# duyhominhnguyen/conan-fgw

Hardware: AMD Instinct MI355X
Metric: molecules/s (K=5 conformers) (higher is better)
Workload: dtype f32

## Files before the change

### conan-fgw_amd/_lib.py

```python
from __future__ import annotations

import ctypes
import os
import subprocess

import torch

_HERE = os.path.dirname(os.path.abspath(__file__))
_SO = os.path.join(_HERE, "libconan_fgw_hip.so")
_LIB = None
ABI_VERSION = 6

c_int, c_float, c_void_p, c_ll = ctypes.c_int, ctypes.c_float, ctypes.c_void_p, ctypes.c_longlong


class FgwParams(ctypes.Structure):
    _fields_ = [("alpha", c_float), ("epsilon", c_float), ("max_iter", c_int), ("tol", c_float), ("inner_tol", c_float),
                ("num_iter_max", c_int), ("stop_thr", c_float), ("fixed_structure", c_int), ("fixed_features", c_int),
                ("warmstart", c_int), ("loss_fun", c_int), ("cs_small_int", c_int)]


class BatchLayout(ctypes.Structure):
    _fields_ = [(n, c_int) for n in ("B", "K", "num_graphs", "num_atoms", "num_bond_edges", "max_nodes", "x_dim", "ea_dim")] + \
               [(n, c_ll) for n in ("off_atom_off", "off_bond_off", "off_z", "off_pos", "off_x", "off_bsrc", "off_bdst", "off_battr", "off_y", "bytes")]


class WgradJob(ctypes.Structure):
    _fields_ = [("ws", c_void_p), ("dW", c_void_p), ("dbias", c_void_p), ("M", c_int), ("K", c_int), ("N", c_int), ("slices", c_int)]


class WgradSlabJob(ctypes.Structure):
    _fields_ = [("g", c_void_p), ("x", c_void_p), ("m_dev", c_void_p), ("ws", c_void_p), ("M", c_int), ("K", c_int), ("N", c_int), ("slices", c_int)]


_P = c_void_p
SIGNATURES = {
    "conan_abi_version": (c_int, []),
    "conan_collate_layout": (c_int, [c_int, c_int, _P, _P, c_int, c_int, ctypes.POINTER(BatchLayout)]),
    "conan_collate_pack": (c_int, [ctypes.POINTER(BatchLayout), _P, _P, _P, _P, _P, _P, _P, _P, _P]),
    "conan_collate_unpack": (c_int, [_P, ctypes.POINTER(BatchLayout), _P, _P, _P, _P, _P, _P, _P, _P, _P, _P, _P]),
    "conan_graph_ptr_from_batch": (c_int, [_P, c_int, c_int, _P, _P]),
    "conan_radius_graph_csr": (c_int, [_P, _P, c_int, c_int, c_float, c_int, c_int, _P, _P, _P, _P, _P, _P]),
    "conan_csr_transpose": (c_int, [_P, c_int, c_int, _P, _P, _P, _P, _P, _P]),
    "conan_edge_pairs": (c_int, [_P, _P, _P, _P, _P, c_int, _P, _P, _P, _P, _P, _P, _P, _P]),
    "conan_radius_graph_build_ws": (c_ll, [c_int, c_int, c_int, c_int]),
    "conan_radius_graph_build": (c_int, [_P, _P, c_int, c_int, c_float, c_int, c_int] + [_P] * 12 + [_P]),
    "conan_edge_index_i64": (c_int, [_P, _P, c_int, _P, _P]),
    "conan_embedding_fwd": (c_int, [_P, _P, c_int, c_int, c_int, _P, _P]),
    "conan_onehot_rows": (c_int, [_P, c_int, c_int, c_int, _P, _P]),
    "conan_embedding_bwd_ws": (c_ll, [c_int, c_int, c_int]),
    "conan_embedding_bwd": (c_int, [_P, _P, c_int, c_int, c_int, c_int, _P, _P, _P]),
    "conan_linear_fwd": (c_int, [_P, _P, _P, _P, c_int, c_int, c_int, c_int, c_int, _P, _P, _P]),
    "conan_linear_multi_fwd": (c_int, [_P, _P, _P, c_int, c_int, c_int, c_int, c_int, _P, _P, _P, _P]),
    "conan_linear_sum_fwd": (c_int, [_P, _P, _P, c_int, c_int, _P, _P, c_int, c_int, _P, _P, _P]),
    "conan_ssp_bwd": (c_int, [_P, _P, c_int, c_int, _P, _P, _P]),
    "conan_linear_wgrad_ws": (c_ll, [c_int, c_int, c_int]),
    "conan_linear_wgrad": (c_int, [_P, _P, c_int, c_int, c_int, _P, _P, _P, _P, _P]),
    "conan_bond_graph_csr": (c_int, [_P, c_int, c_int, _P, _P, _P, _P, _P, _P, _P, _P]),
    "conan_gat_edge_vec": (c_int, [_P, _P, c_int, c_int, _P, _P]),
    "conan_gat_edge_vec_bwd": (c_int, [_P, _P, _P, c_int, c_int, _P, _P, _P]),
    "conan_gat_node_alpha": (c_int, [_P, _P, _P, c_int, c_int, _P, _P, _P]),
    "conan_gat_aggregate_fwd": (c_int, [_P, _P, _P, _P, _P, _P, _P, c_int, _P, _P, c_float, c_int, c_int, _P, _P, _P, _P]),
    "conan_gat_bwd_ws": (c_ll, [c_int, c_int, c_int, c_int]),
    "conan_gat_aggregate_bwd": (c_int, [_P] * 15 + [c_int, _P, c_float, c_int, c_int, c_int, _P, _P, _P, _P]),
    "conan_linear_act_fwd": (c_int, [_P, _P, _P, c_int, c_int, c_int, c_int, _P, _P, _P, _P]),
    "conan_unary_fwd": (c_int, [_P, c_ll, c_int, _P, _P]),
    "conan_unary_bwd": (c_int, [_P, _P, c_ll, c_int, _P, _P]),
    "conan_zero_tail": (c_int, [_P, _P, c_int, c_int, _P]),
    "conan_rbf_wgrad": (c_int, [_P, _P, c_int, _P, c_int, c_float, c_int, _P, _P, _P, _P, _P]),
    "conan_wgrad_batchable": (c_int, [c_int, c_int]),
    "conan_linear_wgrad_scaled": (c_int, [_P, _P, c_int, c_int, c_int, _P, _P, _P, _P, _P, _P]),
    "conan_linear_wgrad_slabs": (c_int, [_P, _P, c_int, c_int, c_int, _P, _P, _P]),
    "conan_rbf_wgrad_slabs": (c_int, [_P, _P, c_int, _P, c_int, c_float, c_int, _P, _P, _P]),
    "conan_wgrad_reduce_batch": (c_int, [ctypes.POINTER(WgradJob), c_int, _P]),
    "conan_linear_wgrad_slabs_batch": (c_int, [ctypes.POINTER(WgradSlabJob), c_int, _P]),
    "conan_filter_bwd_supported": (c_int, [c_int, c_int]),
    "conan_filter_bwd_slices": (c_int, [c_int]),
    "conan_filter_bwd_ws": (c_ll, [c_int, c_int, c_int]),
    "conan_filter_bwd": (c_int, [_P, _P, _P, c_int, _P, c_int, c_float, _P, c_int, _P, _P, _P, _P, _P, _P]),
    "conan_filter_bwd2_supported": (c_int, [c_int, c_int]),
    "conan_filter_bwd2_slices": (c_int, [c_int]),
    "conan_filter_bwd2_ws": (c_ll, [c_int, c_int, c_int]),
    "conan_filter_bwd2": (c_int, [_P, _P, _P, c_int, _P, c_int, c_float, _P, c_int, _P, _P, _P, _P, _P, _P, _P, _P]),
    "conan_rbf_fwd": (c_int, [_P, _P, c_int, _P, c_int, c_float, _P, _P]),
    "conan_cutoff_scale": (c_int, [_P, _P, c_int, c_int, c_float, _P, _P, _P]),
    "conan_stage2_head_supported": (c_int, [c_int]),
    "conan_mse_loss_fwd": (c_int, [_P, _P, c_int, _P, _P, _P]),
    "conan_bce_loss_fwd": (c_int, [_P, _P, _P, c_int, c_int, _P, _P, _P]),
    "conan_stage2_head_fwd": (c_int, [_P, _P, _P, _P, _P, _P, _P, _P, _P, c_float, c_int, c_int, c_int, _P, _P, _P, _P, _P]),
    "conan_stage2_head_bwd": (c_int, [_P, _P, _P, _P, _P, _P, _P, c_float, c_int, c_int, c_int, _P, _P, _P, _P, _P, _P, _P, _P, _P, _P]),
    "conan_stage2_head_sums_supported": (c_int, [c_int, c_int, c_int]),
    "conan_stage2_head_sums_fwd": (c_int, [_P] * 10 + [c_float] + [c_int] * 5 + [_P] * 5),
    "conan_stage2_head_sums_bwd": (c_int, [_P] * 8 + [c_float] + [c_int] * 5 + [_P] * 10),
    "conan_adam_flat_step": (c_int, [_P, _P, _P, _P, _P, _P, c_ll] + [ctypes.c_double] * 5 + [_P, _P]),
    "conan_grad_clip_flat": (c_int, [_P, c_ll, ctypes.c_double, _P, _P, _P, _P]),
    "conan_mlp2_supported": (c_int, [c_int, c_int, c_int, c_int]),
    "conan_mlp2_fwd": (c_int, [_P, _P, _P, _P, _P, _P, c_int, c_int, c_int, c_int, _P, _P, _P]),
    "conan_mlp2_bwd": (c_int, [_P, _P, _P, _P, c_int, c_int, c_int, c_int, _P, _P, _P]),
    "conan_mlp2_outact_supported": (c_int, [c_int, c_int, c_int, c_int]),
    "conan_mlp2_outact_fwd": (c_int, [_P, _P, _P, _P, _P, c_int, c_int, c_int, c_int, _P, _P, _P]),
    "conan_mlp2_outact_bwd": (c_int, [_P, _P, _P, _P, c_int, c_int, c_int, c_int, _P, _P, _P, _P]),
    "conan_mlp2_outact_dual_fwd": (c_int, [_P] * 9 + [c_int] * 4 + [_P, c_int, _P, _P, _P, _P, _P]),
    "conan_mlp2_outact_dual_bwd": (c_int, [_P] * 8 + [c_int] * 4 + [_P, _P, _P, _P, _P, _P, _P]),
    "conan_filter_fused_supported": (c_int, [c_int, c_int]),
    "conan_filter_fwd": (c_int, [_P, _P, c_int, _P, c_int, c_float, c_float, c_int, _P, _P, _P, _P, _P, _P, _P]),
    "conan_filter_cfconv_fwd_supported": (c_int, [c_int, c_int]),
    "conan_filter_cfconv_fwd": (c_int, [_P, _P, _P, _P, _P, c_int, _P, c_int, c_float, c_float, c_int, _P, _P, _P, _P, c_int, _P, _P]),
    "conan_cfconv_fwd": (c_int, [_P, _P, _P, _P, _P, c_int, c_int, _P, _P, _P]),
    "conan_cfconv_bwd_xw_pairs_supported": (c_int, [c_int]),
    "conan_cfconv_bwd_xw_pairs": (c_int, [_P] * 10 + [ctypes.c_float, c_int, c_int, _P, _P, _P, _P]),
    "conan_cfconv_bwd_x": (c_int, [_P, _P, _P, _P, _P, _P, c_int, c_int, _P, _P, _P]),
    "conan_cfconv_bwd_w_pairs": (c_int, [_P, _P, _P, c_int, _P, _P, _P, _P, c_int, _P, c_float, _P, _P, _P]),
    "conan_cfconv_bwd_w": (c_int, [_P, _P, _P, c_int, _P, _P, c_int, _P, c_float, _P, _P]),
    "conan_segment_sum_fwd": (c_int, [_P, _P, c_int, c_int, _P, _P]),
    "conan_segment_sum_bwd": (c_int, [_P, _P, c_int, c_int, _P, _P]),
    "conan_visnet_edge_unit": (c_int, [_P, _P, _P, _P, c_int, _P, _P]),
    "conan_visnet_expnormal": (c_int, [_P, _P, c_int, _P, _P, c_int, c_float, c_float, _P, _P]),
    "conan_visnet_neighbor_scale": (c_int, [_P, _P, _P, _P, _P, c_int, c_int, c_float, _P]),
    "conan_visnet_neighbor_scale_to": (c_int, [_P, _P, _P, _P, _P, c_int, c_int, c_float, _P, _P]),
    "conan_concat2": (c_int, [_P, c_int, _P, c_int, c_ll, _P, _P]),
    "conan_visnet_edge_embed": (c_int, [_P, _P, _P, _P, _P, c_int, c_int, _P, _P]),
    "conan_layernorm_fwd": (c_int, [_P, _P, _P, c_int, c_int, c_float, _P, _P]),
    "conan_scale_channels": (c_int, [_P, _P, c_ll, c_int, _P, _P]),
    "conan_scale_channels_add": (c_int, [_P, _P, _P, c_ll, c_int, _P, _P]),
    "conan_visnet_vecdot": (c_int, [_P, c_int, c_int, _P, _P]),
    "conan_visnet_attn_message": (c_int, [_P, _P, _P, _P, _P, _P, _P, _P, c_float, c_int, c_int, c_int, c_int, _P, _P, _P]),
    "conan_visnet_vec_aggregate": (c_int, [_P, _P, _P, _P, _P, c_int, c_int, c_int, _P, _P]),
    "conan_visnet_node_update": (c_int, [_P, _P, _P, _P, _P, _P, c_int, c_int, _P, _P, _P]),
    "conan_visnet_edge_update": (c_int, [_P, _P, _P, _P, _P, _P, _P, c_int, c_int, c_int, _P, _P, _P]),
    "conan_visnet_spatial_norm": (c_int, [_P, c_int, c_int, _P, _P]),
    "conan_visnet_gate": (c_int, [_P, _P, c_int, c_int, c_int, _P, _P, _P]),
    "conan_visnet_prior": (c_int, [_P, _P, _P, _P, c_int, c_int, _P, _P]),
    "conan_silu_fwd": (c_int, [_P, c_int, c_int, _P, _P, _P]),
    "conan_silu_bwd": (c_int, [_P, _P, c_int, c_int, _P, _P, _P]),
    "conan_split2": (c_int, [_P, c_int, c_int, c_ll, _P, _P, _P]),
    "conan_rowsum": (c_int, [_P, c_int, c_int, _P, _P]),
    "conan_scale_scalar": (c_int, [_P, _P, c_ll, _P, _P]),
    "conan_visnet_edge_embed_bwd": (c_int, [_P, _P, _P, _P, _P, _P, _P, _P, _P, c_int, c_int, c_int, _P, _P, _P]),
    "conan_layernorm_bwd_ws": (c_ll, [c_int, c_int]),
    "conan_layernorm_bwd": (c_int, [_P, _P, _P, c_int, c_int, c_float, _P, _P, _P, _P, _P]),
    "conan_layernorm_bwd_res": (c_int, [_P, _P, _P, _P, c_int, c_int, c_float, _P, _P, _P, _P, _P]),
    "conan_visnet_vecdot_bwd": (c_int, [_P, _P, c_int, c_int, _P, _P]),
    "conan_visnet_attn_message_bwd": (c_int, [_P] * 13 + [c_float, c_int, c_int, c_int, c_int] + [_P] * 6),
    "conan_visnet_vec_aggregate_bwd": (c_int, [_P, _P, _P, _P, _P, _P, _P, _P, _P, c_int, c_int, c_int, c_int, _P, _P, _P]),
    "conan_visnet_node_update_bwd": (c_int, [_P, _P, _P, _P, _P, c_int, c_int, _P, _P, _P, _P]),
    "conan_visnet_edge_update_bwd": (c_int, [_P, _P, _P, _P, _P, _P, _P, _P, _P, _P, c_int, c_int, c_int, _P, _P, _P, _P]),
    "conan_visnet_spatial_norm_bwd": (c_int, [_P, _P, c_int, c_int, _P, _P]),
    "conan_visnet_gate_bwd": (c_int, [_P, _P, _P, _P, c_int, c_int, c_int, _P, _P, _P]),
    "conan_fgw_densify": (c_int, [_P, _P, _P, _P, c_int, c_int, c_int, c_float, c_float, c_float, _P, _P, _P, _P]),
    "conan_fgw_densify_bwd": (c_int, [_P, _P, _P, _P, c_int, c_int, c_int, c_float, c_float, c_float, _P, _P]),
    "conan_fgw_workspace_bytes": (c_ll, [c_int] * 7),
    "conan_fgw_barycenter_fwd": (c_int, [_P, _P, _P, _P, _P, _P, _P, c_int, c_int, c_int, c_int, ctypes.POINTER(FgwParams), c_int, c_int,
                                         _P, _P, _P, _P, _P, _P, _P, _P]),
    "conan_fgw_barycenter_fwd_ragged": (c_int, [_P, _P, _P, _P, _P, _P, _P, _P, _P, _P, c_int, c_int, c_int, c_int, ctypes.POINTER(FgwParams),
                                                c_int, c_int, _P, _P, _P, _P, _P, _P, _P, _P]),
    "conan_fgw_pair_workspace_bytes": (c_ll, [c_int, c_int, c_int, c_int]),
    "conan_fgw_pair_fwd": (c_int, [_P, _P, _P, _P, _P, _P, c_int, c_int, ctypes.POINTER(FgwParams), c_int, c_int, _P, _P, _P, _P, _P, _P]),
    "conan_fgw_pair_dist": (c_int, [_P, _P, _P, _P, _P, _P, c_int, c_int, c_float, c_int, _P, _P]),
    "conan_fgw_pair_dist_bwd": (c_int, [_P, _P, _P, _P, _P, _P, c_int, c_int, c_float, c_int, _P, _P, _P, _P, _P, _P]),
    "conan_fgw_acc_lds_resident": (c_int, [c_int]),
    "conan_fgw_acc_pair_workspace_bytes": (c_ll, [c_int, c_int]),
    "conan_fgw_acc_pair_fwd": (c_int, [_P] * 6 + [c_int, c_int, ctypes.c_double, ctypes.c_double, c_int, ctypes.c_double] + [_P] * 5),
    "conan_fgw_mixup_workspace_bytes": (c_ll, [c_int, c_int, c_int, c_int]),
    "conan_fgw_mixup_barycenter_fwd": (c_int, [_P] * 7 + [c_int, c_int, c_int, c_int, ctypes.POINTER(FgwParams), ctypes.c_double, c_int, ctypes.c_double] + [_P] * 8),
    "conan_sinkhorn_workspace_bytes": (c_ll, [c_int, c_int, c_int]),
    "conan_sinkhorn_lds_resident": (c_int, [c_int, c_int]),
    "conan_sinkhorn_fwd": (c_int, [_P] * 7 + [c_int, c_int, c_int, c_ll, c_float, c_int, c_int, c_float] + [_P] * 8),
    "conan_fgw_barycenter_bwd": (c_int, [_P, _P, _P, _P, c_int, c_int, c_int, c_int, _P, _P]),
    "conan_fgw_barycenter_bwd_full_workspace_bytes": (c_ll, [c_int, c_int, c_int, c_int]),
    "conan_fgw_barycenter_bwd_full": (c_int, [_P, _P, _P, _P, _P, _P, _P, _P, _P, c_int, c_int, c_int, c_int, c_int, c_int, c_int,
                                              _P, _P, _P, _P, _P, _P, _P, _P]),
    "conan_fgw_readout_fwd": (c_int, [_P, c_int, c_int, c_int, c_int, c_int, _P, _P]),
    "conan_fgw_readout_bwd": (c_int, [_P, _P, c_int, c_int, c_int, c_int, c_int, _P, _P]),
}

_ERR = {-1: "bad argument", -2: "HIP launch failure", -3: "unsupported configuration"}


def library_path() -> str:
    return _SO


def build(force: bool = False) -> str:
    args = ["make", "-C", os.path.join(_HERE, "csrc"), "-s", "-j8"]
    if force:
        args.append("-B")
    subprocess.check_call(args)
    return _SO


def lib():
    global _LIB
    if _LIB is None:
        if not os.path.exists(_SO):
            raise RuntimeError(
                f"{_SO} is missing: the HIP extension is not built. Run `python -c 'import __graft_entry__ as g; g.build()'` "
                "(or make -C conan-fgw_amd/csrc). There is no CPU fallback for this path.")
        L = ctypes.CDLL(_SO)
        for name, (res, args) in SIGNATURES.items():
            fn = getattr(L, name)
            fn.restype, fn.argtypes = res, args
        if L.conan_abi_version() != ABI_VERSION:
            raise RuntimeError(f"libconan_fgw_hip.so: ABI version {L.conan_abi_version()} != {ABI_VERSION} expected by _lib.py (stale build: "
                               "make -C conan-fgw_amd/csrc)")
        _LIB = L
    return _LIB


def stream_ptr() -> int:
    return _raw_stream(_cur_device())


try:
    _raw_stream = torch._C._cuda_getCurrentRawStream
    _cur_device = torch._C._cuda_getDevice
except AttributeError:
    def _raw_stream(_dev):
        return torch.cuda.current_stream().cuda_stream

    def _cur_device():
        return torch.cuda.current_device()


def ptr(t, dtype=None):
    if t is None:
        return None
    if not t.is_cuda:
        raise RuntimeError("conan_fgw_amd ops run on the GPU only (got a CPU tensor); there is no CPU fallback")
    if not t.is_contiguous():
        raise RuntimeError("conan_fgw_amd ops need contiguous tensors")
    if dtype is not None and t.dtype != dtype:
        raise RuntimeError(f"expected dtype {dtype}, got {t.dtype}")
    return t.data_ptr()


_TRACE = None


def set_call_trace(fn):
    global _TRACE
    prev, _TRACE = _TRACE, fn
    return prev


def call(name: str, *args):
    fn = getattr(lib(), name)
    rc = fn(*args) if _TRACE is None else _TRACE(name, fn, args)
    if rc != 0:
        raise RuntimeError(f"{name} failed: {_ERR.get(rc, rc)}")
```

### conan-fgw_amd/csrc/fgw.hip

```cpp
#include "fgw_coupling.h"
#ifdef CONAN_FGW_PROFILE
FGW_PROF_ACCESSOR(conan_debug_fgw_prof_large)
FGW_PROF_TRACE_ACCESSOR(conan_debug_fgw_trace_large)
#endif

namespace {

__global__ void k_fgw_init(const float *__restrict__ Cs, const float *__restrict__ init_C, const float *__restrict__ init_Y,
                           FgwDims D, int max_iter, double *__restrict__ Cw, double *__restrict__ Yw, int *__restrict__ active,
                           int *__restrict__ info, float *__restrict__ errs, float *__restrict__ Yout, float *__restrict__ Cout, FgwAdj adj) {
    const int b = blockIdx.x;
    const int NN = D.N * D.N, Nd = D.N * D.d;
    if (!init_C && adj.rowptr) {
        const int N = D.N, g = b * D.K;
        for (int t = threadIdx.x; t < NN; t += blockDim.x) Cout[(size_t)b * NN + t] = 0.f;
        __syncthreads();
        const int lo = adj.gptr[g], n = min(adj.gptr[g + 1] - lo, N);
        for (int e = adj.rowptr[lo] + (int)threadIdx.x; e < adj.rowptr[lo + n]; e += blockDim.x) {
            const int i = adj.tgt[e] - lo, j = adj.col[e] - lo;
            if (i >= 0 && i < N && j >= 0 && j < N) atomicAdd(&Cout[(size_t)b * NN + j * N + i], 1.0f);
        }
        __threadfence_block();
        __syncthreads();
        for (int t = threadIdx.x; t < NN; t += blockDim.x) Cw[(size_t)b * NN + t] = (double)Cout[(size_t)b * NN + t];
    } else {
    const float *c0 = init_C ? init_C + (size_t)b * NN : Cs + (size_t)b * D.K * NN;
    for (int t = threadIdx.x; t < NN; t += blockDim.x) { Cw[(size_t)b * NN + t] = (double)c0[t]; Cout[(size_t)b * NN + t] = c0[t]; }
    }
    for (int t = threadIdx.x; t < Nd; t += blockDim.x) {
        float y = init_Y ? init_Y[(size_t)b * Nd + t] : 0.f;
        Yw[(size_t)b * Nd + t] = (double)y; Yout[(size_t)b * Nd + t] = y;
    }
    if (threadIdx.x == 0) { fgw_active_init(active, D.B, b); info[b * 4 + 0] = 0; info[b * 4 + 1] = 0; info[b * 4 + 2] = 0; info[b * 4 + 3] = 0; }
    for (int t = threadIdx.x; t < 2 * max_iter; t += blockDim.x) errs[(size_t)b * 2 * max_iter + t] = __builtin_nanf("");
    if (adj.order && blockIdx.x == gridDim.x - 1) fgw_order_by_size<256>(adj, D.B, D.K, (int)threadIdx.x);
}

template <int MODE, bool KL, int NW, bool SECOND = false, bool PPA = false, bool ASYM = false>
__global__ void __launch_bounds__(64 * NW) k_fgw_coupling(
    const float *__restrict__ Ys, const float *__restrict__ Cs, const float *__restrict__ ps, const float *__restrict__ pb,
    FgwDims D, conan_fgw_params prm, int outer, int y_zero, const double *__restrict__ Cw, const double *__restrict__ Yw,
    const int *__restrict__ active, float *__restrict__ Tw, int *__restrict__ info, char *__restrict__ scratch,
    fgw_part_t *__restrict__ Ypart, fgw_part_t *__restrict__ Cpart, const int *__restrict__ only, FgwAdj adj) {
    fgw_coupling_solve<MODE, KL, NW, SECOND, PPA, ASYM, false>(Ys, Cs, ps, pb, D, prm, outer, y_zero, Cw, Yw, active, Tw, info, scratch, Ypart, Cpart, only, adj, FgwPair{});
}

#define FGW_MMG mm_f64_glb22
#ifndef CONAN_FGW_ADJ_I8
#define CONAN_FGW_ADJ_I8 1
#endif
template <int NW, bool C2U8, int WPC = 3, bool ORD = false>
__global__ void __launch_bounds__(64 * NW, (NW * WPC + 3) / 4) k_fgw_coupling_big(
    const float *__restrict__ Ys, const float *__restrict__ Cs, const float *__restrict__ ps, const float *__restrict__ pb,
    FgwDims D, conan_fgw_params prm, FastConst fc, int outer, int y_zero, const double *__restrict__ Cw, const double *__restrict__ Yw,
    const int *__restrict__ active, float *__restrict__ Tw, int *__restrict__ info, char *__restrict__ scratch,
    fgw_part_t *__restrict__ Ypart, fgw_part_t *__restrict__ Cpart, int *__restrict__ redo, FgwAdj adj) {
    extern __shared__ __attribute__((aligned(16))) char smem[];
    constexpr int NT = 64 * NW;
    int cid = (gridDim.x & 7) == 0 ? xcd_contiguous_block((int)blockIdx.x, (int)gridDim.x) : (int)blockIdx.x;
    if constexpr (ORD) {
        const int x = (int)blockIdx.x & 7, pblk = (int)blockIdx.x >> 3;
        cid = __builtin_amdgcn_readfirstlane(adj.order[x + 8 * (pblk / D.K)]) * D.K + pblk % D.K;
        asm volatile("" : "+s"(cid));
    }
    const int b = cid / D.K, s = cid % D.K;
    if (!fgw_active(active, D.B, b, outer)) return;
    const int N = D.N, P = D.P, d = D.d;
    const int NN = N * N, NP = N * P;
    const int tid = threadIdx.x, lane = tid & 63, wave = __builtin_amdgcn_readfirstlane(tid >> 6);
    FGW_PROF_DECL;

    float *Kf = reinterpret_cast<float *>(smem);
    double *vec = reinterpret_cast<double *>(smem + (((size_t)NP * 4 + 15) & ~(size_t)15));
    double *fv = vec, *gv = vec + N, *pa = vec + 2 * N, *qb = vec + 3 * N, *refb = vec + 4 * N;
    double *ra = vec + 5 * N, *rb = vec + 6 * N, *y2a = vec + 7 * N, *z2a = vec + 8 * N;
    double *red = vec + 9 * N;
    double *part = red + 16;
    unsigned char *C2b = reinterpret_cast<unsigned char *>(part + NW * N);
    double *bad_flag = red + 15;
    static_assert(NW < 15, "red[15] is the range flag");
    char *gs = scratch + (size_t)cid * coupling_scratch_stride(NP);
    double *Al = reinterpret_cast<double *>(gs) + NP;
    double *base = Al + NP;

    const float *Z = Ys + ((size_t)b * D.K + s) * N * d;
    const float *C2 = Cs + ((size_t)b * D.K + s) * NN;
    const double *C1 = Cw + (size_t)b * NN;
    const double *Y = Yw + (size_t)b * N * d;
    float *Tg = Tw + ((size_t)b * D.K + s) * NN;
    const bool warm = outer > 0 && prm.warmstart;

    int zero_mass = 0;
    for (int i = tid; i < N; i += NT) {
        pa[i] = pb ? (double)pb[(size_t)b * N + i] : fc.inv_n;
        qb[i] = ps ? (double)ps[((size_t)b * D.K + s) * N + i] : fc.inv_n;
        zero_mass |= (pa[i] <= 0.0 || qb[i] <= 0.0) ? 1 : 0;
    }
    if (tid == 0) *bad_flag = 0.0;
    const bool massless = __syncthreads_or(zero_mass) != 0;
    const bool ragged = C2U8 && adj.rowptr != nullptr;
    constexpr bool ADJ_I8 = C2U8 && CONAN_FGW_ADJ_I8 != 0;
    int c2_wide = 0;
    if constexpr (C2U8) {
        for (int t = tid; t < NN; t += NT) {
            const int i = t / N, j = t - i * N;
            const unsigned char cb = ragged ? (unsigned char)0 : (unsigned char)C2[t];
            C2b[i * P + j] = cb;
            c2_wide |= cb > 127 ? 1 : 0;
        }
    }
    const bool adj_i8 = ADJ_I8 && __syncthreads_or(c2_wide) == 0;
    uint4 *Adig = reinterpret_cast<uint4 *>(gs);
    if constexpr (C2U8) {
        if (ragged) {
            __syncthreads();
            adj_scatter_lds_bytes<NT>(adj, cid, N, P, C2b, tid);
            __syncthreads();
        }
    }
    int nb = N, m_pad = 0;
    if constexpr (C2U8) {
        if (ragged) nb = min(adj.gptr[cid + 1] - adj.gptr[cid], N);
        else {
            int mx = 1;
            for (int t = tid; t < NN; t += NT) {
                const int i = t / N, j = t - i * N;
                if (C2b[i * P + j]) mx = max(mx, max(i, j) + 1);
            }
#pragma unroll
            for (int o = 32; o > 0; o >>= 1) mx = max(mx, __shfl_xor(mx, o, 64));
            int *ired = reinterpret_cast<int *>(red);
            if (lane == 0) ired[wave] = mx;
            __syncthreads();
            nb = ired[0];
#pragma unroll
            for (int w = 1; w < NW; ++w) nb = max(nb, ired[w]);
            __syncthreads();
        }
        if (N - nb >= 2 && nb >= 1 && !pb && !ps && !massless && !prm.fixed_structure && !prm.fixed_features) {
            auto near = [](double a, double b_) { return fabs(a - b_) <= 1e-9 * (fabs(b_) + 1e-30) || a == b_; };
            bool ok = true;
            const double cbb = C1[(size_t)nb * N + nb];
            for (int r = nb + 1 + wave; r < N; r += NW) {
                for (int c = lane; c < d; c += 64) {
                    ok = ok && near((double)Z[(size_t)r * d + c], (double)Z[(size_t)nb * d + c]);
                    if (!y_zero) ok = ok && near(Y[(size_t)r * d + c], Y[(size_t)nb * d + c]);
                }
                for (int k = lane; k < N; k += 64) ok = ok && near(C1[(size_t)r * N + k], k < nb ? C1[(size_t)nb * N + k] : cbb);
            }
            for (int k = nb + tid; k < N; k += NT) ok = ok && near(C1[(size_t)nb * N + k], cbb);
            for (int k = wave; k < nb; k += NW)
                for (int c = nb + 1 + lane; c < N; c += 64) ok = ok && near(C1[(size_t)k * N + c], C1[(size_t)k * N + nb]);
            if (__syncthreads_and(ok) != 0) m_pad = N - nb;
// ... 216 lines not shown
                if (r > 0) Yp[(size_t)(nb + r) * d + c] = (fgw_part_t)v;
            }
            __syncthreads();
            for (int c = tid; c < d; c += NT) Yp[(size_t)nb * d + c] = (fgw_part_t)((double)Yp[(size_t)nb * d + c] * im);
        }
    }
    FGW_PROF(9);
    if (!prm.fixed_structure) {
        fgw_part_t *Cp = Cpart + ((size_t)b * D.K + s) * NN;
        if constexpr (C2U8) FGW_MMG<NW, false>(Nx, Nx, Nx, Kf, P, C2b, P, [&](int i, int j, double v) { Al[i * P + j] = v; });
        else FGW_MMG<NW, false>(N, N, N, Kf, P, C2, N, [&](int i, int j, double v) { Al[i * P + j] = v; });
        __syncthreads();
        if (m_pad) {
            FGW_MMG<NW, true>(Nx, Nx, Nx, Al, P, Kf, P, [&](int i, int j, double v) { base[i * P + j] = v; });
            __threadfence_block();
            __syncthreads();
            const double im = 1.0 / mult;
            for (int t = tid; t < NN; t += NT) {
                const int i = t / N, j = t - i * N;
                Cp[t] = (fgw_part_t)(base[min(i, nb) * P + min(j, nb)] * ((i >= nb ? im : 1.0) * (j >= nb ? im : 1.0)));
            }
        } else {
            FGW_MMG<NW, true>(N, N, N, Al, P, Kf, P, [&](int i, int j, double v) { Cp[i * N + j] = (fgw_part_t)v; });
        }
    }
    FGW_PROF(10);
    FGW_PROF_FLUSH;
    FGW_PROF_TRACE(Nx | (cpt << 8) | (sk_total << 20));
}

template <bool LDS>
__global__ void __launch_bounds__(256) k_fgw_bwd(const float *__restrict__ T, const float *__restrict__ dY, const float *__restrict__ pb,
                                                 const float *__restrict__ lambdas, int K, int N, int d, float *__restrict__ dYs) {
    extern __shared__ float bw_smem[];
    const int b = blockIdx.x / K, s = blockIdx.x % K;
    const float *Ts = T + ((size_t)b * K + s) * N * N;
    const float *g = dY + (size_t)b * N * d;
    const float lam = lambdas ? lambdas[s] : 1.0f / (float)K;
    if (LDS) {
        float *Tl = bw_smem, *gl = bw_smem + N * N;
        for (int t = threadIdx.x; t < N * N; t += 256) Tl[t] = Ts[t];
        for (int t = threadIdx.x; t < N * d; t += 256) {
            const int i = t / d;
            const float pinv = pb ? (pb[(size_t)b * N + i] > 0.f ? 1.0f / pb[(size_t)b * N + i] : 0.f) : (float)N;
            gl[t] = pinv * g[t];
        }
        __syncthreads();
        for (int t = threadIdx.x; t < N * d; t += 256) {
            const int j = t / d, c = t - j * d;
            float a = 0.f;
            for (int i = 0; i < N; ++i) a += Tl[i * N + j] * gl[i * d + c];
            dYs[((size_t)b * K + s) * N * d + t] = lam * a;
        }
        return;
    }
    for (int t = threadIdx.x; t < N * d; t += 256) {
        const int j = t / d, c = t - j * d;
        float a = 0.f;
        for (int i = 0; i < N; ++i) {
            const float pinv = pb ? (pb[(size_t)b * N + i] > 0.f ? 1.0f / pb[(size_t)b * N + i] : 0.f) : (float)N;
            a += Ts[i * N + j] * pinv * g[i * d + c];
        }
        dYs[((size_t)b * K + s) * N * d + t] = lam * a;
    }
}

__global__ void __launch_bounds__(256) k_densify(const float *__restrict__ feat, const int *__restrict__ gptr, const int *__restrict__ rowptr,
                                                 const int *__restrict__ col, int N, int d, float shift, float a, float b,
                                                 float *__restrict__ Ys, float *__restrict__ Cs, float *__restrict__ minmax) {
    __shared__ float smn[4], smx[4];
    const int g = blockIdx.x;
    const int lo = gptr[g], n_raw = gptr[g + 1] - lo;
    const bool overflow = n_raw > N;
    const int n = overflow ? N : n_raw;
    const int tid = threadIdx.x;
    float mn = 3.0e38f, mx = -3.0e38f;
    for (int t = tid; t < n * d; t += 256) { const float v = feat[(size_t)lo * d + t] + shift; mn = fminf(mn, v); mx = fmaxf(mx, v); }
    if (n < N) { const float v = 0.f + shift; mn = fminf(mn, v); mx = fmaxf(mx, v); }
    mn = wave_min(mn); mx = wave_max(mx);
    if ((tid & 63) == 0) { smn[tid >> 6] = mn; smx[tid >> 6] = mx; }
    __syncthreads();
    mn = fminf(fminf(smn[0], smn[1]), fminf(smn[2], smn[3]));
    mx = fmaxf(fmaxf(smx[0], smx[1]), fmaxf(smx[2], smx[3]));
    if (overflow) mn = mx = __builtin_nanf("");
    if (tid == 0) { minmax[g * 2] = mn; minmax[g * 2 + 1] = mx; }
    const float scale = b - a, range = mx - mn;
    float *Yg = Ys + (size_t)g * N * d;
    for (int t = tid; t < N * d; t += 256) {
        const float x = (t < n * d ? feat[(size_t)lo * d + t] : 0.f) + shift;
        Yg[t] = a + __fdiv_rn((x - mn) * scale, range);
    }
    if (!Cs) return;
    float *Cg = Cs + (size_t)g * N * N;
    for (int t = tid; t < N * N; t += 256) Cg[t] = 0.f;
    __syncthreads();
    __shared__ int rp[257];
    const int e0 = rowptr[lo], e1 = rowptr[lo + n];
    for (int i0 = 0; i0 < n; i0 += 256) {
        const int m = min(256, n - i0);
        __syncthreads();
        for (int t = tid; t <= m; t += 256) rp[t] = rowptr[lo + i0 + t];
        __syncthreads();
        for (int e = rp[0] + tid; e < rp[m]; e += 256) {
            int a = 0, b = m;
            while (b - a > 1) { const int c = (a + b) >> 1; if (rp[c] <= e) a = c; else b = c; }
            const int i = i0 + a, j = col[e] - lo;
            if (j >= 0 && j < N) atomicAdd(&Cg[j * N + i], 1.0f);
        }
    }
    (void)e0; (void)e1;
}

__global__ void __launch_bounds__(256) k_adj_dense(FgwAdj adj, int N) { (void)adj_dense_slice<256>(adj, (int)blockIdx.x, N, (int)threadIdx.x); }

__global__ void __launch_bounds__(256) k_densify_bwd(const float *__restrict__ feat, const float *__restrict__ dYs, const int *__restrict__ gptr,
                                                     const float *__restrict__ minmax, int N, int d, float shift, float a, float b,
                                                     float *__restrict__ dfeat) {
    __shared__ float red[3][4];
    const int g = blockIdx.x;
    const int lo = gptr[g], n_raw = gptr[g + 1] - lo;
    const int n = n_raw > N ? N : n_raw;
    const int tid = threadIdx.x;
    const float mn = minmax[g * 2], mx = minmax[g * 2 + 1];
    const float s = b - a, r = mx - mn;
    const float *G = dYs + (size_t)g * N * d;
    float s0 = 0.f, s1 = 0.f, cmin = 0.f, cmax = 0.f;
    for (int t = tid; t < N * d; t += 256) {
        const float x = (t < n * d ? feat[(size_t)lo * d + t] : 0.f) + shift;
        const float gg = G[t];
        s0 += gg; s1 += gg * (x - mn);
        cmin += (x == mn) ? 1.f : 0.f; cmax += (x == mx) ? 1.f : 0.f;
    }
    float vals[4] = {s0, s1, cmin, cmax};
    __shared__ float tot[4];
    for (int q = 0; q < 4; ++q) {
        float v = wave_sum(vals[q]);
        if ((tid & 63) == 0) red[0][tid >> 6] = v;
        __syncthreads();
        if (tid == 0) tot[q] = red[0][0] + red[0][1] + red[0][2] + red[0][3];
        __syncthreads();
    }
    const float dmn = -tot[0] * s / r + tot[1] * s / (r * r);
    const float dmx = -tot[1] * s / (r * r);
    for (int t = tid; t < n * d; t += 256) {
        const float x = feat[(size_t)lo * d + t] + shift;
        float gx = G[t] * s / r;
        if (x == mn) gx += dmn / tot[2];
        if (x == mx) gx += dmx / tot[3];
        dfeat[(size_t)lo * d + t] = gx;
    }
    for (int t = n * d + tid; t < n_raw * d; t += 256) dfeat[(size_t)lo * d + t] = __builtin_nanf("");
}

__global__ void __launch_bounds__(64) k_readout_fwd(const float *__restrict__ Y, int K, int N, int d, int mode, float *__restrict__ out) {
    const int b = blockIdx.x;
    const float *Yb = Y + (size_t)b * N * d;
    __shared__ int has_nan;
    if (threadIdx.x == 0) has_nan = 0;
    __syncthreads();
    if (mode == 1) {
        int bad = 0;
        for (int t = threadIdx.x; t < N * d; t += 64) bad |= isnan(Yb[t]) ? 1 : 0;
        if (bad) has_nan = 1;
        __syncthreads();
    }
    for (int c = threadIdx.x; c < d; c += 64) {
        float sum = 0.f, sq = 0.f;
        for (int i0 = 0; i0 < N; i0 += 8) {
            float v[8];
#pragma unroll
            for (int u = 0; u < 8; ++u) v[u] = Yb[min(i0 + u, N - 1) * d + c];
#pragma unroll
            for (int u = 0; u < 8; ++u) { const float y = (has_nan || i0 + u >= N) ? 0.f : v[u]; sum += y; sq += y * y; }
        }
        float r = mode == 1 ? sum / sqrtf(sq) : sum;
        for (int k = 0; k < K; ++k) out[((size_t)b * K + k) * d + c] = r;
    }
}
__global__ void __launch_bounds__(64) k_readout_bwd(const float *__restrict__ Y, const float *__restrict__ dout, int K, int N, int d, int mode,
                                                    float *__restrict__ dY) {
    const int b = blockIdx.x;
    const float *Yb = Y + (size_t)b * N * d;
    for (int c = threadIdx.x; c < d; c += 64) {
        float g = 0.f;
        for (int k = 0; k < K; ++k) g += dout[((size_t)b * K + k) * d + c];
        if (mode == 0) {
            for (int i = 0; i < N; ++i) dY[((size_t)b * N + i) * d + c] = g;
        } else {
            float sum = 0.f, sq = 0.f;
            for (int i = 0; i < N; ++i) { const float y = Yb[i * d + c]; sum += y; sq += y * y; }
            const float nrm = sqrtf(sq);
            for (int i = 0; i < N; ++i) dY[((size_t)b * N + i) * d + c] = g * (1.0f / nrm - sum * Yb[i * d + c] / (nrm * nrm * nrm));
        }
    }
}

#ifndef CONAN_FGW_WPC2_MAX
#define CONAN_FGW_WPC2_MAX 512
#endif
#ifndef CONAN_FGW_WPC2_ORDERED
#define CONAN_FGW_WPC2_ORDERED 1
#endif
#ifndef CONAN_FGW_BIG_ORDER
#define CONAN_FGW_BIG_ORDER 1
#endif
#ifndef CONAN_FGW_BIG_WPC2
#define CONAN_FGW_BIG_WPC2 1
#endif
constexpr bool BIG_WPC2 = CONAN_FGW_BIG_WPC2 != 0;
inline size_t big_lds(int N, bool c2_bytes) {
    return (((size_t)N * pitch_of(N) * 4 + 15) & ~(size_t)15) + (size_t)((9 + GEN_NW) * N + 16) * 8 + (c2_bytes ? (size_t)N * pitch_of(N) : 0);
}

FgwWorkspace fgw_workspace(int B, int K, int N, int d, bool ragged, int solver, int symmetric) {
    FgwWorkspace w{};
    if (B <= 0 || K <= 0 || N <= 0 || d <= 0 || solver < 0 || solver > 2 || symmetric < -1 || symmetric > 1) return w;
    const size_t NN = (size_t)N * N, NP = (size_t)N * pitch_of(N), BK = (size_t)B * K;
    size_t end = 0;
    auto region = [&](size_t bytes) { const size_t at = end; end += bytes; return at; };
    w.Cw = region(al256((size_t)B * NN * 8));
    w.Yw = region(al256((size_t)B * N * d * 8));
    w.active = region(al256((size_t)B * 16));
    w.scratch = region(al256(BK * coupling_scratch_stride(NP)));
    w.order = region(al256((size_t)B * NP * 16));
    w.Ypart = region(BK * N * d * sizeof(fgw_part_t));
    w.Cpart = region(BK * NN * sizeof(fgw_part_t));
    end = (end + 15) & ~(size_t)15;
    w.zvec = region(BK * 2 * N * 8);
    w.yvec = region((size_t)B * 2 * N * 8);
    w.redo = region(BK * 4 + 512);
    w.dense = region(ragged ? al256(BK * NN * sizeof(float)) : 0);
    w.asym = region(solver == 2 && symmetric != 1 ? al256(conan_fgw_bapg_asym_scratch_bytes(B, K, N)) : 0);
    w.total = end;
    return w;
}

enum class FgwPath {
    Small,
    Big,
    General,
    Bapg
};
struct FgwPlan {
    FgwPath path;
    int mode;
    size_t lds_bytes;
    bool kl, ppa, asym;
    bool y_from_t;
    size_t big_bytes;
    bool big_u8, big_wpc2, big_ordered;
};

template <int M>
void launch_general(const FgwCall &c, const FgwPlan &pl, int outer, int y_zero, const int *only) {
    auto go = [&](auto kernel, int blocks) {
        launch_lds(kernel, blocks, 64 * GEN_NW, pl.lds_bytes, c.s, c.Ys, c.Cs, c.ps, c.p, c.D, c.prm, outer, y_zero | (c.symmetric < 0 ? 2 : 0), c.Cw,
                   c.Yw, c.active, c.T, c.info, c.scratch, c.Ypart, c.Cpart, only, c.adj);
    };
    if (only) go(k_fgw_coupling<M, false, GEN_NW, true>, (c.D.B * c.D.K + 63) / 64);
    else with_flags([&](auto KL, auto PPA, auto ASYM) { go(k_fgw_coupling<M, KL.value, GEN_NW, false, PPA.value, ASYM.value>, c.D.B * c.D.K); },
                    pl.kl, pl.ppa, pl.asym);
}

int fgw_fwd_impl(const float *Ys, const float *Cs, const float *ps, const float *p, const float *lambdas, const float *init_C,
                 const float *init_Y, int B, int K, int N, int d, const conan_fgw_params *params, float *Y, float *C, float *T, float *T_iter,
                 int *info, float *errs, void *workspace, void *stream, FgwAdj adj, int solver, int symmetric) {
    if (solver < 0 || solver > 2 || symmetric < -1 || symmetric > 1) return CONAN_E_BADARG;
    if (!Ys || !(Cs || (adj.gptr && adj.rowptr && adj.col && adj.tgt)) || !params || !Y || !C || !T || !info || !errs || !workspace || B <= 0 || K <= 0 || N <= 0 || d <= 0)
        return CONAN_E_BADARG;
    if (params->max_iter <= 0 || params->num_iter_max <= 0) return CONAN_E_BADARG;
    if (params->fixed_features && !init_Y) return CONAN_E_BADARG;
    if (params->loss_fun != 0 && params->loss_fun != 1) return CONAN_E_BADARG;
    const bool ragged = adj.rowptr != nullptr, small = conan_fgw_small_supported(N, d), kl = params->loss_fun != 0;
    const bool model = solver == 0 && symmetric == 1;
    const FgwWorkspace w = fgw_workspace(B, K, N, d, ragged, solver, symmetric);
    const size_t NN = (size_t)N * N, NP = (size_t)N * pitch_of(N);
    FgwCall c{};
    c.Ys = Ys; c.Cs = Cs; c.ps = ps; c.p = p; c.lambdas = lambdas; c.init_C = init_C; c.init_Y = init_Y;
    c.D = FgwDims{B, K, N, d, pitch_of(N)};
    c.prm = *params;
    c.adj = adj;
    c.symmetric = symmetric;
    c.Y = Y; c.C = C; c.T = T; c.info = info; c.errs = errs;
    c.Cw = ws_at<double>(workspace, w.Cw); c.Yw = ws_at<double>(workspace, w.Yw); c.active = ws_at<int>(workspace, w.active);
    c.scratch = ws_at<char>(workspace, w.scratch); c.scratch_stride = coupling_scratch_stride(NP);
    c.Ypart = ws_at<fgw_part_t>(workspace, w.Ypart); c.Cpart = ws_at<fgw_part_t>(workspace, w.Cpart);
    c.redo = ws_at<int>(workspace, w.redo);
    c.asym_scratch = ws_at<char>(workspace, w.asym);
    c.s = as_stream(stream);
    if (ragged) {
        c.prm.cs_small_int = 1;
        c.adj.dense = ws_at<float>(workspace, w.dense);
        if (!(model && !kl && (small ? conan_fgw_fast_supported(N, d, 1) : big_lds(N, true) <= LDS_LIMIT))) {
            k_adj_dense<<<B * K, 256, 0, c.s>>>(c.adj, N);
            c.Cs = c.adj.dense;
            c.adj.rowptr = nullptr;
        }
    }
    if (!model) c.adj = FgwAdj{};
    if (c.adj.rowptr && !kl && (B & 7) == 0 && B <= 4096 && (small || (CONAN_FGW_BIG_ORDER && big_lds(N, true) <= LDS_LIMIT)))
        c.adj.order = ws_at<int>(workspace, w.order);

    FgwPlan pl{};
    pl.kl = kl; pl.ppa = solver == 1; pl.asym = symmetric != 1;
    pl.big_u8 = c.prm.cs_small_int != 0;
    pl.big_bytes = big_lds(N, pl.big_u8);
    pl.path = solver == 2 ? FgwPath::Bapg : model && small ? FgwPath::Small : model && !kl && pl.big_bytes <= LDS_LIMIT ? FgwPath::Big : FgwPath::General;
    pl.mode = general_mode(N, &pl.lds_bytes);
    pl.big_wpc2 = BIG_WPC2 && (B * K <= CONAN_FGW_WPC2_MAX || (CONAN_FGW_WPC2_ORDERED && c.adj.order));
    pl.big_ordered = c.adj.order != nullptr && (B * K & 7) == 0 && pl.big_wpc2 && pl.big_u8;
    pl.y_from_t = pl.path == FgwPath::Small && !c.prm.fixed_features && conan_fgw_update_chunk(K, N, d, B) > 0;
    if (pl.path == FgwPath::Small) { c.zvec = ws_at<double>(workspace, w.zvec); c.yvec = ws_at<double>(workspace, w.yvec); }

    if (pl.path == FgwPath::Small) conan_fgw_small_prepare(c);
    else k_fgw_init<<<B, 256, 0, c.s>>>(c.Cs, init_C, init_Y, c.D, c.prm.max_iter, c.Cw, c.Yw, c.active, info, errs, Y, C, c.adj);
    const FastConst fc = fast_const(c.prm, N);
    for (int outer = 0; outer < c.prm.max_iter; ++outer) {
        const int y_zero = (outer == 0 && !init_Y) ? 1 : 0;
        const int *only = nullptr;
        if (pl.path == FgwPath::Big) {
            auto big = [&](auto kernel) {
                launch_lds(kernel, B * K, 64 * GEN_NW, pl.big_bytes, c.s, c.Ys, c.Cs, c.ps, c.p, c.D, c.prm, fc, outer, y_zero, c.Cw, c.Yw, c.active, c.T,
                           c.info, c.scratch, c.Ypart, c.Cpart, c.redo, c.adj);
            };
            if (pl.big_ordered) big(k_fgw_coupling_big<GEN_NW, true, 2, true>);
            else if (pl.big_u8) { if (pl.big_wpc2) big(k_fgw_coupling_big<GEN_NW, true, 2, false>); else big(k_fgw_coupling_big<GEN_NW, true, 3, false>); }
            else { if (pl.big_wpc2) big(k_fgw_coupling_big<GEN_NW, false, 2, false>); else big(k_fgw_coupling_big<GEN_NW, false, 3, false>); }
            only = c.redo;
        }
        if (pl.path == FgwPath::Small) conan_fgw_small_coupling(c, outer, y_zero, pl.y_from_t ? nullptr : c.Ypart);
        else if (pl.path == FgwPath::Bapg) conan_fgw_bapg_coupling(c, outer, y_zero);
        else if (pl.mode == 2) launch_general<2>(c, pl, outer, y_zero, only);
        else if (pl.mode == 1) launch_general<1>(c, pl, outer, y_zero, only);
        else launch_general<0>(c, pl, outer, y_zero, only);
        if (T_iter)
            (void)hipMemcpyAsync(T_iter + (size_t)outer * B * K * NN, T, (size_t)B * K * NN * sizeof(float), hipMemcpyDeviceToDevice, c.s);
        conan_fgw_small_update(c, outer, pl.y_from_t);
    }
    CONAN_LAUNCH_CHECK();
    return CONAN_OK;
}

}

extern "C" {

long long conan_fgw_workspace_bytes(int B, int K, int N, int d, int ragged, int solver, int symmetric) {
    if (ragged != 0 && ragged != 1) return 0;
    return (long long)fgw_workspace(B, K, N, d, ragged != 0, solver, symmetric).total;
}

int conan_fgw_barycenter_fwd(const float *Ys, const float *Cs, const float *ps, const float *p, const float *lambdas,
                             const float *init_C, const float *init_Y, int B, int K, int N, int d,
                             const conan_fgw_params *params, int solver, int symmetric, float *Y, float *C, float *T, float *T_iter,
                             int *info, float *errs, void *workspace, void *stream) {
    return fgw_fwd_impl(Ys, Cs, ps, p, lambdas, init_C, init_Y, B, K, N, d, params, Y, C, T, T_iter, info, errs, workspace, stream, FgwAdj{}, solver,
                        symmetric);
}

int conan_fgw_barycenter_fwd_ragged(const float *Ys, const int *graph_ptr, const int *rowptr, const int *col, const int *tgt, const float *ps,
                                    const float *p, const float *lambdas, const float *init_C, const float *init_Y, int B, int K, int N, int d,
                                    const conan_fgw_params *params, int solver, int symmetric, float *Y, float *C, float *T, float *T_iter,
                                    int *info, float *errs, void *workspace, void *stream) {
    return fgw_fwd_impl(Ys, nullptr, ps, p, lambdas, init_C, init_Y, B, K, N, d, params, Y, C, T, T_iter, info, errs, workspace, stream,
                        FgwAdj{graph_ptr, rowptr, col, tgt, nullptr, nullptr}, solver, symmetric);
}

int conan_fgw_barycenter_bwd(const float *T, const float *dY, const float *p, const float *lambdas, int B, int K,
                             int N, int d, float *dYs, void *stream) {
    if (!T || !dY || !dYs || B <= 0 || K <= 0 || N <= 0 || d <= 0) return CONAN_E_BADARG;
    const size_t bw_lds = ((size_t)N * N + (size_t)N * d) * sizeof(float);
    if (bw_lds <= 64 * 1024) k_fgw_bwd<true><<<B * K, 256, bw_lds, as_stream(stream)>>>(T, dY, p, lambdas, K, N, d, dYs);
    else k_fgw_bwd<false><<<B * K, 256, 0, as_stream(stream)>>>(T, dY, p, lambdas, K, N, d, dYs);
    CONAN_LAUNCH_CHECK();
    return CONAN_OK;
}

int conan_fgw_densify(const float *feat, const int *graph_ptr, const int *rowptr, const int *col, int num_graphs,
                      int N, int d, float shift, float a, float b, float *Ys, float *Cs, float *minmax, void *stream) {
    if (!feat || !graph_ptr || !Ys || !minmax || num_graphs <= 0 || N <= 0 || d <= 0 || (Cs && (!rowptr || !col))) return CONAN_E_BADARG;
    k_densify<<<num_graphs, 256, 0, as_stream(stream)>>>(feat, graph_ptr, rowptr, col, N, d, shift, a, b, Ys, Cs, minmax);
    CONAN_LAUNCH_CHECK();
    return CONAN_OK;
}

int conan_fgw_densify_bwd(const float *feat, const float *dYs, const int *graph_ptr, const float *minmax,
                          int num_graphs, int N, int d, float shift, float a, float b, float *dfeat, void *stream) {
    if (!feat || !dYs || !graph_ptr || !minmax || !dfeat || num_graphs <= 0 || N <= 0 || d <= 0) return CONAN_E_BADARG;
    k_densify_bwd<<<num_graphs, 256, 0, as_stream(stream)>>>(feat, dYs, graph_ptr, minmax, N, d, shift, a, b, dfeat);
    CONAN_LAUNCH_CHECK();
    return CONAN_OK;
}

int conan_fgw_readout_fwd(const float *Y, int B, int K, int N, int d, int mode, float *out, void *stream) {
    if (!Y || !out || B <= 0 || K <= 0 || N <= 0 || d <= 0 || mode < 0 || mode > 1) return CONAN_E_BADARG;
    k_readout_fwd<<<B, 64, 0, as_stream(stream)>>>(Y, K, N, d, mode, out);
    CONAN_LAUNCH_CHECK();
    return CONAN_OK;
}

int conan_fgw_readout_bwd(const float *Y, const float *dout, int B, int K, int N, int d, int mode, float *dY,
                          void *stream) {
    if (!Y || !dout || !dY || B <= 0 || K <= 0 || N <= 0 || d <= 0 || mode < 0 || mode > 1) return CONAN_E_BADARG;
    k_readout_bwd<<<B, 64, 0, as_stream(stream)>>>(Y, dout, K, N, d, mode, dY);
    CONAN_LAUNCH_CHECK();
    return CONAN_OK;
}

}
```

### conan-fgw_amd/csrc/fgw_common.h

```cpp
#pragma once
#include <type_traits>
#include "common.h"

#ifdef CONAN_FGW_PROFILE
static __device__ long long g_fgw_prof[32];
#define FGW_PROF_ACCESSOR(name)                                                          \
    extern "C" int name(long long *out, int reset) {                                     \
        if (out && hipMemcpyFromSymbol(out, HIP_SYMBOL(g_fgw_prof), sizeof(long long) * 32) != hipSuccess) return -2; \
        if (reset) { long long z[32] = {0}; if (hipMemcpyToSymbol(HIP_SYMBOL(g_fgw_prof), z, sizeof(z)) != hipSuccess) return -2; } \
        return 0;                                                                        \
    }
static __device__ long long g_fgw_trace[2 + 6 * 8192];
#define FGW_PROF_TRACE_ACCESSOR(name)                                                    \
    extern "C" int name(long long *out, int reset) {                                     \
        if (out && hipMemcpyFromSymbol(out, HIP_SYMBOL(g_fgw_trace), sizeof(long long) * (2 + 6 * 8192)) != hipSuccess) return -2; \
        if (reset) { long long z[2] = {0, 0}; if (hipMemcpyToSymbol(HIP_SYMBOL(g_fgw_trace), z, sizeof(z)) != hipSuccess) return -2; } \
        return 0;                                                                        \
    }
#define FGW_PROF_TRACE(tag)                                                              \
    do {                                                                                 \
        if (threadIdx.x == 0) {                                                          \
            const unsigned long long i_ = atomicAdd(reinterpret_cast<unsigned long long *>(&g_fgw_trace[0]), 1ull); \
            if (i_ < 8192) {                                                             \
                long long *r_ = &g_fgw_trace[2 + 6 * i_];                                \
// ... 99 lines not shown
    const double t = x * 1.4426950408889634074;
    const double n = rint(t);
    const float f = (float)(t - n);
    const float e = __builtin_amdgcn_exp2f(f);
    return ldexp((double)e, (int)n);
}

__device__ __forceinline__ double exp_fast(double x) {
    const double xc = fmin(fmax(x, -700.0), 700.0);
    const double t = xc * 1.4426950408889634074;
    const double sh = t + 6755399441055744.0;
    const int n = __double2loint(sh);
    const double f = t - (sh - 6755399441055744.0);
    const double e = (double)__builtin_amdgcn_exp2f((float)f);
    const double scale = __hiloint2double((n + 1023) << 20, 0);
    const double r = e * scale;
    return x > -700.0 ? (x < 700.0 ? r : __builtin_inf()) : 0.0;
}

__device__ __forceinline__ double rcp_pos(double s) {
    double r = __builtin_amdgcn_rcp(s);
    r = fma(fma(-s, r, 1.0), r, r);
    r = fma(fma(-s, r, 1.0), r, r);
    return r;
}

__device__ __forceinline__ double log_acc(double s) {
    const double y0 = (double)(__builtin_amdgcn_logf((float)s) * 0.693147180559945309f);
    const double r = s * exp_acc(-y0) - 1.0;
    return y0 + (r - 0.5 * r * r);
}

__device__ __forceinline__ double wave_sum_d(double v) {
#pragma unroll
    for (int o = 32; o > 0; o >>= 1) v += __shfl_xor(v, o, 64);
    return v;
}
__device__ __forceinline__ double wave_max_d(double v) {
#pragma unroll
    for (int o = 32; o > 0; o >>= 1) { double w = __shfl_xor(v, o, 64); v = w > v ? w : v; }
    return v;
}

template <int NW = FGW_WAVES>
__device__ __forceinline__ double block_sum_d(double v, double *red) {
    v = wave_sum_d(v);
    __syncthreads();
    if ((threadIdx.x & 63) == 0) red[threadIdx.x >> 6] = v;
    __syncthreads();
    double s = 0.0;
#pragma unroll
    for (int w = 0; w < NW; ++w) s += red[w];
    return s;
}


typedef double f64x4 __attribute__((ext_vector_type(4)));

__device__ __forceinline__ double exp_lse(double x) {
    const float f = (float)x;
    return (double)__builtin_amdgcn_exp2f(f * 1.44269504088896340736f);
}

template <int NW = FGW_WAVES, class FX, class FW, class FS>
__device__ __forceinline__ void mm_f64_pad(int M, int Nn, int Kd, FX X, FW W, FS st) {
    const int lane = threadIdx.x & 63, wave = __builtin_amdgcn_readfirstlane((int)(threadIdx.x >> 6));
    const int Mq = (M + 15) >> 4, Nq = (Nn + 15) >> 4;
    const int li = lane & 15, lk = lane >> 4;
    for (int t = wave; t < Mq * Nq; t += NW) {
        const int i0 = (t / Nq) << 4, j0 = (t % Nq) << 4;
        const int ia = i0 + li, jb = j0 + li;
        const bool ra = ia < M, cb = jb < Nn;
        const int ic = ra ? ia : M - 1, jc = cb ? jb : Nn - 1;
        f64x4 acc = {0.0, 0.0, 0.0, 0.0};
        int k0 = 0;
        for (; k0 + 16 <= Kd; k0 += 16) {
            double a[4], b[4];
#pragma unroll
            for (int u = 0; u < 4; ++u) { a[u] = X(ic, k0 + 4 * u + lk); b[u] = W(k0 + 4 * u + lk, jc); }
#pragma unroll
            for (int u = 0; u < 4; ++u) acc = __builtin_amdgcn_mfma_f64_16x16x4f64(ra ? a[u] : 0.0, cb ? b[u] : 0.0, acc, 0, 0, 0);
        }
        if (k0 < Kd) {
            double a[4], b[4];
#pragma unroll
            for (int u = 0; u < 4; ++u) {
                const int k = k0 + 4 * u + lk, kc = k < Kd ? k : Kd - 1;
                a[u] = X(ic, kc); b[u] = W(kc, jc);
            }
#pragma unroll
            for (int u = 0; u < 4; ++u) {
                const bool kin = k0 + 4 * u + lk < Kd;
                if (k0 + 4 * u < Kd)
                    acc = __builtin_amdgcn_mfma_f64_16x16x4f64((ra && kin) ? a[u] : 0.0, (cb && kin) ? b[u] : 0.0, acc, 0, 0, 0);
            }
        }
#pragma unroll
        for (int q = 0; q < 4; ++q) {
            const int i = i0 + lk + 4 * q;
            if (i < M && cb) st(i, jb, acc[q]);
        }
    }
}

template <int NW, bool WT, typename TX, typename TW, class FS>
__device__ __forceinline__ void mm_f64_glb(int M, int Nn, int Kd, const TX *__restrict__ X, int pX, const TW *__restrict__ W, int pW, FS st,
                                           const int tid = threadIdx.x) {
    const int lane = tid & 63, wave = __builtin_amdgcn_readfirstlane(tid >> 6);
    const int Mq = (M + 15) >> 4, Nq = (Nn + 15) >> 4;
    const int li = lane & 15, lk = lane >> 4;
    for (int t = wave; t < Mq * Nq; t += NW) {
        const int i0 = (t / Nq) << 4, j0 = (t % Nq) << 4;
        const int ia = i0 + li, jb = j0 + li;
        const bool ra = ia < M, cb = jb < Nn;
        const TX *xr = X + (size_t)(ra ? ia : M - 1) * pX;
        const int jc = cb ? jb : Nn - 1;
        f64x4 acc = {0.0, 0.0, 0.0, 0.0}, acc2 = {0.0, 0.0, 0.0, 0.0};
        for (int k0 = 0; k0 < Kd; k0 += 16) {
            const int kb = k0 + 4 * lk;
            double a[4], b[4];
            if (k0 + 16 <= Kd) {
#pragma unroll
                for (int u = 0; u < 4; ++u) a[u] = (double)xr[kb + u];
                if (WT) {
                    const TW *wr = W + (size_t)jc * pW + kb;
#pragma unroll
                    for (int u = 0; u < 4; ++u) b[u] = (double)wr[u];
                } else {
#pragma unroll
                    for (int u = 0; u < 4; ++u) b[u] = (double)W[(size_t)(kb + u) * pW + jc];
                }
            } else {
#pragma unroll
                for (int u = 0; u < 4; ++u) {
                    const int k = kb + u, kc = k < Kd ? k : Kd - 1;
                    const double av = (double)xr[kc], bv = (double)(WT ? W[(size_t)jc * pW + kc] : W[(size_t)kc * pW + jc]);
                    a[u] = k < Kd ? av : 0.0; b[u] = k < Kd ? bv : 0.0;
                }
            }
            acc = __builtin_amdgcn_mfma_f64_16x16x4f64(ra ? a[0] : 0.0, cb ? b[0] : 0.0, acc, 0, 0, 0);
            acc2 = __builtin_amdgcn_mfma_f64_16x16x4f64(ra ? a[1] : 0.0, cb ? b[1] : 0.0, acc2, 0, 0, 0);
            acc = __builtin_amdgcn_mfma_f64_16x16x4f64(ra ? a[2] : 0.0, cb ? b[2] : 0.0, acc, 0, 0, 0);
            acc2 = __builtin_amdgcn_mfma_f64_16x16x4f64(ra ? a[3] : 0.0, cb ? b[3] : 0.0, acc2, 0, 0, 0);
        }
#pragma unroll
        for (int q = 0; q < 4; ++q) {
            const int i = i0 + lk + 4 * q;
            if (i < M && cb) st(i, jb, acc[q] + acc2[q]);
        }
    }
}

template <int NT>
__device__ __forceinline__ void fgw_order_by_size(const FgwAdj &adj, int B, int K, int tid) {
    static_assert(NT >= 256, "one thread per size bin");
    __shared__ unsigned char nsz[4096];
    __shared__ int hist[256], base[256];
    if (B > 4096) return;
    for (int t = tid; t < 256; t += NT) hist[t] = 0;
    __syncthreads();
    for (int m = tid; m < B; m += NT) {
        const int n = min(max(adj.gptr[m * K + 1] - adj.gptr[m * K], 0), 255);
        nsz[m] = (unsigned char)n;
        atomicAdd(&hist[n], 1);
    }
    __syncthreads();
    if (tid == 0) {
        int run = 0;
        for (int v = 255; v >= 0; --v) { base[v] = run; run += hist[v]; }
    }
    __syncthreads();
    if (tid < 256 && hist[tid] > 0) {
        int pos = base[tid];
        for (int m = 0; m < B; ++m)
            if (nsz[m] == (unsigned char)tid) adj.order[pos++] = m;
    }
}

#ifndef CONAN_FGW_KT
#define CONAN_FGW_KT 2
#endif
template <int NW, bool WT, typename TX, typename TW, class FS, int KT = CONAN_FGW_KT>
__device__ __forceinline__ void mm_f64_glb22(int M, int Nn, int Kd, const TX *__restrict__ X, int pX, const TW *__restrict__ W, int pW, FS st,
                                             const int tid = threadIdx.x) {
    const int lane = tid & 63, wave = __builtin_amdgcn_readfirstlane(tid >> 6);
    const int Mq = (M + 15) >> 4, Nq = (Nn + 15) >> 4;
    const int li = lane & 15, lk = lane >> 4;
    const int Mb = Mq >> 1, Nb = Nq >> 1;
    const int nblk = Mb * Nb, nblk_used = (nblk / NW) * NW;
    auto load_a = [&](const TX *xr, int kb, int k0, double (&a)[KT]) {
        if (k0 + 4 * KT <= Kd) {
#pragma unroll
            for (int u = 0; u < KT; ++u) a[u] = (double)xr[kb + u];
        } else {
#pragma unroll
            for (int u = 0; u < KT; ++u) { const int k = kb + u; const double v = (double)xr[k < Kd ? k : Kd - 1]; a[u] = k < Kd ? v : 0.0; }
        }
    };
    auto load_b = [&](int jc, int kb, int k0, double (&b)[KT]) {
        if (k0 + 4 * KT <= Kd) {
#pragma unroll
            for (int u = 0; u < KT; ++u) b[u] = (double)(WT ? W[(size_t)jc * pW + kb + u] : W[(size_t)(kb + u) * pW + jc]);
        } else {
#pragma unroll
            for (int u = 0; u < KT; ++u) {
                const int k = kb + u, kc = k < Kd ? k : Kd - 1;
                const double v = (double)(WT ? W[(size_t)jc * pW + kc] : W[(size_t)kc * pW + jc]);
                b[u] = k < Kd ? v : 0.0;
            }
        }
    };
    auto store_tile = [&](int i0, int j0, const f64x4 &r) {
        const int jb = j0 + li;
        if (jb < Nn) {
#pragma unroll
            for (int q = 0; q < 4; ++q) { const int i = i0 + lk + 4 * q; if (i < M) st(i, jb, r[q]); }
        }
    };
    for (int t = wave; t < nblk_used; t += NW) {
        const int i0 = (t / Nb) << 5, j0 = (t % Nb) << 5;
        const TX *x0 = X + (size_t)min(i0 + li, M - 1) * pX, *x1 = X + (size_t)min(i0 + 16 + li, M - 1) * pX;
        const int jc0 = min(j0 + li, Nn - 1), jc1 = min(j0 + 16 + li, Nn - 1);
        f64x4 c00 = {0.0, 0.0, 0.0, 0.0}, c01 = c00, c10 = c00, c11 = c00;
        for (int k0 = 0; k0 < Kd; k0 += 4 * KT) {
            const int kb = k0 + KT * lk;
            double a0[KT], a1[KT], b0[KT], b1[KT];
            load_a(x0, kb, k0, a0); load_a(x1, kb, k0, a1); load_b(jc0, kb, k0, b0); load_b(jc1, kb, k0, b1);
#pragma unroll
            for (int u = 0; u < KT; ++u) {
                c00 = __builtin_amdgcn_mfma_f64_16x16x4f64(a0[u], b0[u], c00, 0, 0, 0);
                c01 = __builtin_amdgcn_mfma_f64_16x16x4f64(a0[u], b1[u], c01, 0, 0, 0);
                c10 = __builtin_amdgcn_mfma_f64_16x16x4f64(a1[u], b0[u], c10, 0, 0, 0);
                c11 = __builtin_amdgcn_mfma_f64_16x16x4f64(a1[u], b1[u], c11, 0, 0, 0);
            }
        }
        store_tile(i0, j0, c00); store_tile(i0, j0 + 16, c01); store_tile(i0 + 16, j0, c10); store_tile(i0 + 16, j0 + 16, c11);
    }
    const int rest_blk = nblk - nblk_used;
    const int n_single = rest_blk * 4 + (Mq * Nq - 4 * nblk);
    for (int t = wave; t < n_single; t += NW) {
        int ti, tj;
        if (t < rest_blk * 4) { const int bq = nblk_used + (t >> 2); ti = 2 * (bq / Nb) + ((t >> 1) & 1); tj = 2 * (bq % Nb) + (t & 1); }
        else {
            int q = t - rest_blk * 4;
            const int ncol = (Nq & 1) ? Mq : 0;
            if (q < ncol) { ti = q; tj = Nq - 1; }
            else { q -= ncol; ti = Mq - 1; tj = q; }
        }
        const int i0 = ti << 4, j0 = tj << 4;
        const TX *xr = X + (size_t)min(i0 + li, M - 1) * pX;
        const int jc = min(j0 + li, Nn - 1);
        f64x4 acc = {0.0, 0.0, 0.0, 0.0}, acc2 = {0.0, 0.0, 0.0, 0.0};
        for (int k0 = 0; k0 < Kd; k0 += 4 * KT) {
            const int kb = k0 + KT * lk;
            double a[KT], bq[KT];
            load_a(xr, kb, k0, a); load_b(jc, kb, k0, bq);
#pragma unroll
            for (int u = 0; u < KT; ++u) {
                if (u & 1) acc2 = __builtin_amdgcn_mfma_f64_16x16x4f64(a[u], bq[u], acc2, 0, 0, 0);
                else acc = __builtin_amdgcn_mfma_f64_16x16x4f64(a[u], bq[u], acc, 0, 0, 0);
            }
        }
        store_tile(i0, j0, acc + acc2);
    }
}

typedef int fgw_i32x4 __attribute__((ext_vector_type(4)));
__device__ __forceinline__ void fgw_digit_planes4(const double (&v)[4], double scale, unsigned (&pl)[4]) {
    unsigned r[4];
#pragma unroll
    for (int u = 0; u < 4; ++u) r[u] = ((unsigned)__double2int_rn(v[u] * scale) + 0x00808080u) ^ 0x00808080u;
    const unsigned t0 = __builtin_amdgcn_perm(r[1], r[0], 0x05010400u), t1 = __builtin_amdgcn_perm(r[1], r[0], 0x07030602u);
    const unsigned t2 = __builtin_amdgcn_perm(r[3], r[2], 0x05010400u), t3 = __builtin_amdgcn_perm(r[3], r[2], 0x07030602u);
    pl[0] = __builtin_amdgcn_perm(t2, t0, 0x05040100u); pl[1] = __builtin_amdgcn_perm(t2, t0, 0x07060302u);
    pl[2] = __builtin_amdgcn_perm(t3, t1, 0x05040100u); pl[3] = __builtin_amdgcn_perm(t3, t1, 0x07060302u);
}
template <int NT>
__device__ __forceinline__ void fgw_digits_from_f64(int M, int Kd, const double *__restrict__ X, int pX, int xexp, uint4 *__restrict__ D, const int tid = threadIdx.x) {
    const int KB = ((Kd + 31) >> 5) << 2;
    const double scale = __longlong_as_double((long long)(1023 + 31 - xexp) << 52);
    constexpr int R = 2;
    for (int base = 0; base < M * KB; base += R * NT) {
        double v[R][8];
#pragma unroll
        for (int q = 0; q < R; ++q) {
            const int idx = base + q * NT + tid;
            const int ic = idx < M * KB ? idx : M * KB - 1;
            const int i = ic / KB, kb = ic - i * KB;
            const double *xr = X + (size_t)i * pX;
#pragma unroll
            for (int u = 0; u < 8; ++u) { const int k = 8 * kb + u; v[q][u] = xr[k < Kd ? k : Kd - 1]; }
        }
#pragma unroll
        for (int q = 0; q < R; ++q) {
            const int idx = base + q * NT + tid;
            if (idx >= M * KB) continue;
            const int kb = idx % KB;
            double v0[4], v1[4];
#pragma unroll
            for (int u = 0; u < 4; ++u) { v0[u] = 8 * kb + u < Kd ? v[q][u] : 0.0; v1[u] = 8 * kb + 4 + u < Kd ? v[q][4 + u] : 0.0; }
            unsigned lo[4], hi[4];
            fgw_digit_planes4(v0, scale, lo); fgw_digit_planes4(v1, scale, hi);
            D[2 * idx] = make_uint4(lo[0], hi[0], lo[1], hi[1]);
            D[2 * idx + 1] = make_uint4(lo[2], hi[2], lo[3], hi[3]);
        }
    }
}
__device__ __forceinline__ long fgw_bytes8(const unsigned char *__restrict__ w, int kb, int Kd) {
    unsigned lo = 0, hi = 0;
#pragma unroll
    for (int u = 0; u < 4; ++u) {
        const int k0 = kb + u, k1 = kb + 4 + u;
        lo |= (unsigned)w[k0 < Kd ? k0 : Kd - 1] << (8 * u);
        hi |= (unsigned)w[k1 < Kd ? k1 : Kd - 1] << (8 * u);
    }
    return (long)(((unsigned long long)hi << 32) | lo);
}
template <int NW, class FS>
__device__ __forceinline__ void mm_adj_i8(int M, int Nn, int Kd, const uint4 *__restrict__ D, const unsigned char *__restrict__ Wb, int pW, int xexp, FS st,
                                          const int tid = threadIdx.x) {
// ... 365 lines not shown
        const int ws = WT ? S : S * pW;
        int k0 = 0;
        double p0 = 0.0, p1 = 0.0;
        for (; k0 + 8 <= nfull; k0 += 8) {
            double xa[8], wb[8];
#pragma unroll
            for (int u = 0; u < 8; ++u) { xa[u] = (double)xp[S * u]; wb[u] = (double)wp[u * ws]; }
            xp += 8 * S; wp += 8 * ws;
#pragma unroll
            for (int u = 0; u < 8; u += 2) { p0 = fma(xa[u], wb[u], p0); p1 = fma(xa[u + 1], wb[u + 1], p1); }
        }
        for (; k0 < nfull; ++k0) { p0 = fma((double)xp[0], (double)wp[0], p0); xp += S; wp += ws; }
        if (rem) {
            const int back = sub < rem ? 0 : sub;
            double xt = (double)xp[-back];
            const double wt = (double)(WT ? wp[-back] : wp[-back * pW]);
            xt = sub < rem ? xt : 0.0;
            p1 = fma(xt, wt, p1);
        }
        acc = p0 + p1;
    }
    return acc;
}

template <int NW, int MAXT, int KMAX, bool WT, bool HOLD, typename TX, typename TW, class FM, class FS>
__device__ __forceinline__ void mm_lds2(int M, int Nn, int Kd, const TX *__restrict__ X, int pX, const TW *__restrict__ W, int pW, FM mid, FS st,
                                        const int tid = threadIdx.x) {
    const int lane = tid & 63, wave = __builtin_amdgcn_readfirstlane(tid >> 6);
    const int li = lane & 15, lk = lane >> 4;
    const bool border = border_path<NW>(M, Nn);
    const int Mq = border ? M >> 4 : (M + 15) >> 4, Nq = border ? Nn >> 4 : (Nn + 15) >> 4;
    auto tile = [&](int t) {
        const int i0 = (t / Nq) << 4, j0 = (t % Nq) << 4;
        const int ia = i0 + li, jb = j0 + li;
        const bool ra = ia < M, cb = jb < Nn;
        const TX *xp = X + (ra ? ia : M - 1) * pX + lk;
        const TW *wp = WT ? W + (cb ? jb : Nn - 1) * pW + lk : W + lk * pW + (cb ? jb : Nn - 1);
        return mm2_tile<KMAX, WT>(xp, wp, pW, Kd, lk);
    };
    auto store_tile = [&](int t, const f64x4 &r) {
        const int i0 = (t / Nq) << 4, j0 = (t % Nq) << 4, jb = j0 + li;
        if (jb < Nn) {
#pragma unroll
            for (int q = 0; q < 4; ++q) {
                const int i = i0 + lk + 4 * q;
                if (i < M) st(i, jb, r[q]);
            }
        }
    };
    f64x4 res[HOLD ? MAXT : 1];
    if constexpr (HOLD) {
#pragma unroll
        for (int tt = 0; tt < MAXT; ++tt) {
            const int t = wave + tt * NW;
            res[tt] = f64x4{0.0, 0.0, 0.0, 0.0};
            if (t < Mq * Nq) res[tt] = tile(t);
        }
    } else {
        for (int t = wave; t < Mq * Nq; t += NW) store_tile(t, tile(t));
    }
    const int Mc = (M >> 4) << 4, Nc = (Nn >> 4) << 4, nb1 = (M - Mc) * Nn;
    const int bcount = border ? nb1 + Mc * (Nn - Nc) : 0;
    const bool thin = bcount <= NW * 21;
    double bval[2] = {0.0, 0.0};
    int b_i[2] = {0, 0}, b_j[2] = {0, 0};
    bool b_on[2] = {false, false};
    auto border_ij = [&](int o, int &bi, int &bj) {
        if (o < nb1) { bi = Mc + o / Nn; bj = o % Nn; }
        else { const int q = o - nb1; bi = q / (Nn - Nc); bj = Nc + q % (Nn - Nc); }
    };
    if (border && thin) {
        const int o = wave * 21 + lane / 3, sub3 = lane % 3;
        const bool on = lane < 63 && o < bcount;
        if (on) border_ij(o, b_i[0], b_j[0]);
        double acc = 0.0;
        if (on) {
            const TX *xp = X + b_i[0] * pX + sub3;
            const TW *wp = WT ? W + b_j[0] * pW + sub3 : W + sub3 * pW + b_j[0];
            acc = mm2_border_part<KMAX, 3, WT>(xp, wp, pW, Kd, sub3);
        }
        const double a1 = __shfl(acc, lane + 1, 64), a2 = __shfl(acc, lane + 2, 64);
        bval[0] = acc + a1 + a2;
        b_on[0] = on && sub3 == 0;
    } else if (border) {
        const int sub = tid & 3;
#pragma unroll
        for (int p = 0; p < 2; ++p) {
            if (p * (NW * 16) >= bcount) break;
            const int o = p * (NW * 16) + (tid >> 2);
            const bool on = o < bcount;
            if (on) border_ij(o, b_i[p], b_j[p]);
            double acc = 0.0;
            if (on) {
                const TX *xp = X + b_i[p] * pX + sub;
                const TW *wp = WT ? W + b_j[p] * pW + sub : W + sub * pW + b_j[p];
                acc = mm2_border_part<KMAX, 4, WT>(xp, wp, pW, Kd, sub);
            }
            acc += __shfl_xor(acc, 1, 64);
            acc += __shfl_xor(acc, 2, 64);
            bval[p] = acc;
            b_on[p] = on && sub == 0;
        }
    }
    mid();
    if constexpr (HOLD) {
#pragma unroll
        for (int tt = 0; tt < MAXT; ++tt) {
            const int t = wave + tt * NW;
            if (t < Mq * Nq) store_tile(t, res[tt]);
        }
    }
#pragma unroll
    for (int p = 0; p < 2; ++p)
        if (b_on[p]) st(b_i[p], b_j[p], bval[p]);
}


struct FgwWorkspace {
    size_t Cw, Yw, active, scratch, order, Ypart, Cpart, zvec, yvec, redo, dense, asym, total;
};
struct FgwPairWorkspace {
    size_t C1w, scratch, total, stride;
};
struct FgwPairCall {
    const float *M, *C2, *p, *q;
    const double *C1w;
    FgwDims D;
    conan_fgw_params prm;
    int symmetric, warm;
    float *T;
    int *info;
    FgwPair pr;
    char *scratch;
    size_t scratch_stride;
    hipStream_t s;
};

struct FgwCall {
    const float *Ys, *Cs, *ps, *p, *lambdas, *init_C, *init_Y;
    FgwDims D;
    conan_fgw_params prm;
    FgwAdj adj;
    int symmetric;
    float *Y, *C, *T;
    int *info;
    float *errs;
    double *Cw, *Yw;
    int *active;
    char *scratch;
    size_t scratch_stride;
    fgw_part_t *Ypart, *Cpart;
    double *zvec, *yvec;
    int *redo;
    char *asym_scratch;
    hipStream_t s;
};

template <class... KA, class... A>
inline void launch_lds(void (*kernel)(KA...), int grid, int block, size_t lds, hipStream_t s, A &&...args) {
    if (lds > 64 * 1024) (void)hipFuncSetAttribute(reinterpret_cast<const void *>(kernel), hipFuncAttributeMaxDynamicSharedMemorySize, (int)lds);
    kernel<<<grid, block, lds, s>>>(static_cast<KA>(args)...);
}
template <class F>
inline void with_flags(F &&f) { f(); }
template <class F, class... B>
inline void with_flags(F &&f, bool b, B... rest) {
    if (b) with_flags([&](auto... c) { f(std::true_type{}, c...); }, rest...);
    else with_flags([&](auto... c) { f(std::false_type{}, c...); }, rest...);
}

namespace {
__host__ __device__ inline size_t coupling_scratch_stride(size_t NP) { return (NP * 28 + 15) / 16 * 16; }
inline int pitch_of(int N) { return fgw_pitch(N); }
inline size_t al256(size_t v) { return (v + 255) / 256 * 256; }
constexpr int GEN_NW = 8;
inline size_t coupling_lds(int N) { return (size_t)((6 + 2 * GEN_NW) * N + 16) * 8 + (size_t)N * pitch_of(N) * 28; }
constexpr size_t LDS_LIMIT = 160 * 1024;
inline int general_mode(int N, size_t *lds_bytes) {
    const size_t lc = coupling_lds(N), vec_c = (size_t)((6 + 2 * GEN_NW) * N + 16) * 8, mr_bytes = (size_t)N * pitch_of(N) * 8;
    const int mode = lc <= LDS_LIMIT ? 2 : (vec_c + mr_bytes <= LDS_LIMIT ? 1 : 0);
    *lds_bytes = mode == 2 ? lc : vec_c + (mode == 1 ? mr_bytes : 0);
    return mode;
}
template <class T>
inline T *ws_at(void *workspace, size_t offset) { return reinterpret_cast<T *>(static_cast<char *>(workspace) + offset); }
}
#ifndef CONAN_FGW_ASYM_C1T
#define CONAN_FGW_ASYM_C1T 1
#endif

bool conan_fgw_small_supported(int N, int d);
bool conan_fgw_fast_supported(int N, int d, int small_int);
void conan_fgw_small_prepare(const FgwCall &c);
void conan_fgw_small_coupling(const FgwCall &c, int outer, int y_zero, fgw_part_t *Ypart);
void conan_fgw_small_update(const FgwCall &c, int outer, bool y_from_t);
int conan_fgw_update_chunk(int K, int N, int d, int B);
size_t conan_fgw_bapg_lds(int N, bool asym = false);
size_t conan_fgw_bapg_asym_scratch_bytes(int B, int K, int N);
void conan_fgw_bapg_coupling(const FgwCall &c, int outer, int y_zero);
size_t conan_fgw_bapg_pair_stride(int N, bool asym);
void conan_fgw_bapg_pair(const FgwPairCall &c);
```

### conan-fgw_amd/csrc/fgw_small.hip

```cpp
#include "fgw_common.h"

#ifdef CONAN_FGW_PROFILE
FGW_PROF_ACCESSOR(conan_debug_fgw_prof)
FGW_PROF_TRACE_ACCESSOR(conan_debug_fgw_trace)
#endif

namespace {

constexpr int SK_SCRATCH_DOUBLES = 3 * 256 + 2 * 64;

template <int R, bool KL, bool SECOND = false>
__global__ void __launch_bounds__(FGW_THREADS, (SECOND || R > 9) ? 1 : 3) k_fgw_coupling_small(
    const float *__restrict__ Ys, const float *__restrict__ Cs, const float *__restrict__ ps, const float *__restrict__ pb,
    FgwDims D, conan_fgw_params prm, int outer, int y_zero, const double *__restrict__ Cw, const double *__restrict__ Yw,
    const int *__restrict__ active, float *__restrict__ Tw, int *__restrict__ info, fgw_part_t *__restrict__ Ypart,
    fgw_part_t *__restrict__ Cpart, const double *__restrict__ zvec, const double *__restrict__ yvec, const int *__restrict__ only, FgwAdj adj) {
    extern __shared__ __attribute__((aligned(16))) char smem[];
    auto solve = [&](const int cid) {
    const int b = cid / D.K, s = cid % D.K;
    if (!fgw_active(active, D.B, b, outer)) return;
    const int N = D.N, P = D.P, d = D.d;
    const int NN = N * N, NP = N * P;
    const int tid = threadIdx.x, lane = tid & 63, w = __builtin_amdgcn_readfirstlane(tid >> 6);
    const bool lane_ok = lane < N;
// ... 681 lines not shown
            g = lq_ok ? pi_l * rcp_pos(rs) : 0.0;
            gvP[permL] = g;
            if (ii % 10 == 0) {
                *bufCw = dotR(kA, gw);
                __syncthreads();
                colp = ((bufC[lq] + bufC[64 + lq]) + bufC[128 + lq]) + bufC[192 + lq];
                have_colp = true;
                double df = lq_ok ? f * colp - qj : 0.0;
                df = df * df;
                if (lq == nbq) df /= (double)m_pad;
                df = wave_sum_d(df);
                if (sqrt(df) < fc.stop_thr) { ++ii; break; }
            }
        }
        if (bail) break;
        sk_total += ii;
        FGW_PROF(6);
        double e2 = 0.0;
        {
            float *trow = Tl + wq * P + lq;
#pragma unroll
            for (int r = 0; r < R; ++r) {
                const bool ok = lq_ok && wq + 4 * r < N;
                float *tp = ok ? trow + 4 * r * P : t_dummy;
                const float tn = (float)((gw[r] * kA[r]) * f);
                double df = ok ? (double)tn - (double)*tp : 0.0;
                df *= df;
                if (nbq >= 0) {
                    const double im = 1.0 / (double)m_pad;
                    df *= (lq == nbq ? im : 1.0) * (wq + 4 * r == nbq ? im : 1.0);
                }
                e2 += df;
                *tp = tn;
            }
        }
        if (cpt % 10 == 0) err = sqrt(block_sum_d(e2, red));
        else __syncthreads();
        ++cpt;
        FGW_PROF(7);
    }
    if (bail) {
        if (tid == 0) { redo[cid] = 1; atomicOr(&info[b * 4 + 3], 1); }
        return;
    }
    __syncthreads();
    {
        int te = tid;
        asm volatile("" : "+v"(te));
        int i = te / N, j = te - i * N;
        const int dq = FGW_THREADS / N, dr = FGW_THREADS - dq * N;
        if (m_pad) {
            const float im = (float)(1.0 / mult);
            for (int t = te; t < NN; t += FGW_THREADS) {
                Tg[t] = Tl[min(i, nb) * P + min(j, nb)] * ((i >= nb ? im : 1.0f) * (j >= nb ? im : 1.0f));
                j += dr; i += dq;
                if (j >= N) { j -= N; ++i; }
            }
        } else {
            for (int t = te; t < NN; t += FGW_THREADS) {
                Tg[t] = Tl[i * P + j];
                j += dr; i += dq;
                if (j >= N) { j -= N; ++i; }
            }
        }
    }
    if (tid == 0) { atomicAdd(&info[b * 4 + 1], cpt); atomicAdd(&info[b * 4 + 2], sk_total); redo[cid] = 0; if (m_pad) atomicOr(&info[b * 4 + 3], 2); }
    FGW_PROF(8);

    if (!prm.fixed_features && Ypart) {
        fgw_part_t *Yp = Ypart + ((size_t)b * D.K + s) * N * d;
        if (yz_lds) {
            const int Nd = N * d;
            for (int t0 = tid; t0 < Nd; t0 += 4 * FGW_THREADS) {
                float zv[4];
#pragma unroll
                for (int u = 0; u < 4; ++u) { const int t = t0 + u * FGW_THREADS; zv[u] = Z[t < Nd ? t : Nd - 1]; }
#pragma unroll
                for (int u = 0; u < 4; ++u) { const int t = t0 + u * FGW_THREADS; if (t < Nd) Zl[t] = zv[u]; }
            }
            __syncthreads();
            mm_lds2<FGW_WAVES, 1, 0, false, false>(N, d, N, Tl, P, Zl, d, [] {}, [&](int i, int c, double v) { Yp[(size_t)i * d + c] = (fgw_part_t)v; });
        } else {
            mm_f64(N, d, N, [&](int i, int k) { return (double)Tl[i * P + k]; }, [&](int k, int c) { return (double)Z[(size_t)k * d + c]; },
                   [&](int i, int c, double v) { Yp[(size_t)i * d + c] = (fgw_part_t)v; });
        }
    }
    FGW_PROF(9);
    if (!prm.fixed_structure) {
        fgw_part_t *Cp = Cpart + ((size_t)b * D.K + s) * NN;
        if (complete) {
            {
                const int lc = lane < Nx ? lane : Nx - 1;
                const float *tr = Tl + lc * P + w;
                double p0 = 0.0, p1 = 0.0;
#pragma unroll
                for (int r = 0; r < R; ++r) {
                    const int q = w + 4 * r;
                    if (q < n_real) { if (r & 1) p1 += (double)tr[4 * r]; else p0 += (double)tr[4 * r]; }
                }
                if (lane < Nx) rsum[w * N + lane] = p0 + p1;
            }
            __syncthreads();
            mm_lds2<FGW_WAVES, 1, 0, true, false>(Nx, Nx, n_real, Tl, P, Tl, P, [] {}, [&](int i, int j, double v) {
                const double ti = ((rsum[i] + rsum[N + i]) + rsum[2 * N + i]) + rsum[3 * N + i];
                const double tj = ((rsum[j] + rsum[N + j]) + rsum[2 * N + j]) + rsum[3 * N + j];
                if (m_pad) Bl[i * P + j] = ti * tj - v;
                else Cp[i * N + j] = (fgw_part_t)(ti * tj - v);
            });
        } else {
            mm_lds2<FGW_WAVES, 1, 0, false, false>(Nx, Nx, Nx, Tl, P, C2l, P, [] {}, [&](int i, int j, double v) { AKl[i * P + j] = v; });
            __syncthreads();
            mm_lds2<FGW_WAVES, 1, 0, true, false>(Nx, Nx, Nx, AKl, P, Tl, P, [] {}, [&](int i, int j, double v) {
                if (m_pad) Bl[i * P + j] = v;
                else Cp[i * N + j] = (fgw_part_t)v;
            });
        }
        if (m_pad) {
            __syncthreads();
            const double im = 1.0 / mult;
            int i = tid / N, j = tid - i * N;
            const int dq = FGW_THREADS / N, dr = FGW_THREADS - dq * N;
            for (int t = tid; t < NN; t += FGW_THREADS) {
                Cp[t] = (fgw_part_t)(Bl[min(i, nb) * P + min(j, nb)] * ((i >= nb ? im : 1.0) * (j >= nb ? im : 1.0)));
                j += dr; i += dq;
                if (j >= N) { j -= N; ++i; }
            }
        }
    }
    FGW_PROF(10);
    FGW_PROF_FLUSH;
    FGW_PROF_TRACE(Nx | (cpt << 8) | (sk_total << 20));
}

template <int NT>
__device__ __forceinline__ void molecule_vectors(const double *__restrict__ Y, const double *__restrict__ C, const float *__restrict__ p, int N,
                                                 int d, bool kl, double *__restrict__ out, int which = 2) {
    constexpr int LPI = NT / 64;
    const int i = (int)threadIdx.x / LPI, sub = (int)threadIdx.x % LPI;
    double y2 = 0.0, r1 = 0.0;
    if (i < N) {
        if (which != 1)
            for (int c = sub; c < d; c += LPI) { const double v = Y[(size_t)i * d + c]; y2 += v * v; }
        if (which != 0)
            for (int k = sub; k < N; k += LPI) {
                const double c1 = C[i * N + k], pk = p ? (double)p[k] : 1.0 / (double)N;
                r1 += (kl ? c1 * log(c1 + 1e-15) - c1 : c1 * c1) * pk;
            }
    }
#pragma unroll
    for (int o = 1; o < LPI; o <<= 1) { y2 += __shfl_xor(y2, o, 64); r1 += __shfl_xor(r1, o, 64); }
    if (i < N && sub == 0) { if (which != 1) out[i] = y2; if (which != 0) out[N + i] = r1; }
}

__global__ void __launch_bounds__(256) k_fgw_small_vectors(const float *__restrict__ Ys, const float *__restrict__ Cs, const float *__restrict__ ps,
                                                           const float *__restrict__ pb, FgwDims D, int kl, double *__restrict__ Cw,
                                                           double *__restrict__ Yw, double *__restrict__ zvec, double *__restrict__ yvec,
                                                           const float *__restrict__ init_C, const float *__restrict__ init_Y, int max_iter,
                                                           int *__restrict__ active, int *__restrict__ info, float *__restrict__ errs,
                                                           float *__restrict__ Yout, float *__restrict__ Cout, FgwAdj adj) {
    const int b = blockIdx.x / D.K, s = blockIdx.x % D.K;
    const int N = D.N, d = D.d;
    __shared__ __attribute__((aligned(16))) unsigned char cm[64 * 65 + 16];
    const int Pm = D.P;
    if (adj.rowptr) {
        for (int t = threadIdx.x; t < (64 * 65 + 16) / 4; t += 256) reinterpret_cast<unsigned *>(cm)[t] = 0u;
        __syncthreads();
        adj_scatter_lds_bytes<256>(adj, (int)blockIdx.x, N, Pm, cm, (int)threadIdx.x);
        __syncthreads();
    }
    if (s == 0) {
        const int NN = N * N, Nd = N * d;
        const float *c0 = init_C ? init_C + (size_t)b * NN : Cs + (size_t)b * D.K * NN;
        for (int t = threadIdx.x; t < NN; t += 256) {
            const float cv = (!init_C && adj.rowptr) ? (float)cm[(t / N) * Pm + (t % N)] : c0[t];
            Cw[(size_t)b * NN + t] = (double)cv; Cout[(size_t)b * NN + t] = cv;
        }
        for (int t = threadIdx.x; t < Nd; t += 256) {
            const float y = init_Y ? init_Y[(size_t)b * Nd + t] : 0.f;
            Yw[(size_t)b * Nd + t] = (double)y; Yout[(size_t)b * Nd + t] = y;
        }
        if (threadIdx.x == 0) { fgw_active_init(active, D.B, b); info[b * 4 + 0] = 0; info[b * 4 + 1] = 0; info[b * 4 + 2] = 0; info[b * 4 + 3] = 0; }
        for (int t = threadIdx.x; t < 2 * max_iter; t += 256) errs[(size_t)b * 2 * max_iter + t] = __builtin_nanf("");
        __syncthreads();
    }
    const float *Z = Ys + ((size_t)b * D.K + s) * N * d;
    const float *C2 = Cs + ((size_t)b * D.K + s) * N * N;
    const float *q = ps ? ps + ((size_t)b * D.K + s) * N : nullptr;
    const int j = (int)threadIdx.x >> 2, sub = (int)threadIdx.x & 3;
    double z2 = 0.0, r2 = 0.0;
    if (j < N) {
        for (int c = sub; c < d; c += 4) { const double v = (double)Z[(size_t)j * d + c]; z2 += v * v; }
        for (int k = sub; k < N; k += 4) {
            const double c2 = adj.rowptr ? (double)cm[j * Pm + k] : (double)C2[j * N + k], qk = q ? (double)q[k] : 1.0 / (double)N;
            r2 += qk * (kl ? c2 : c2 * c2);
        }
    }
    z2 += __shfl_xor(z2, 1, 64); z2 += __shfl_xor(z2, 2, 64);
    r2 += __shfl_xor(r2, 1, 64); r2 += __shfl_xor(r2, 2, 64);
    double *zo = zvec + ((size_t)b * D.K + s) * 2 * N;
    if (j < N && sub == 0) { zo[j] = z2; zo[N + j] = r2; }
    if (s == 0)
        molecule_vectors<256>(Yw + (size_t)b * N * d, Cw + (size_t)b * N * N, pb ? pb + (size_t)b * N : nullptr, N, d, kl != 0, yvec + (size_t)b * 2 * N);
    if (adj.order && blockIdx.x == gridDim.x - 1) fgw_order_by_size<256>(adj, D.B, D.K, (int)threadIdx.x);
}

constexpr int UPD_THREADS = 512;
template <bool Y_FROM_T>
__global__ void __launch_bounds__(UPD_THREADS) k_fgw_update_parts(
    const float *__restrict__ pb, const float *__restrict__ lambdas, FgwDims D, conan_fgw_params prm, int outer,
    const fgw_part_t *__restrict__ Ypart, const fgw_part_t *__restrict__ Cpart, double *__restrict__ Cw, double *__restrict__ Yw,
    int *__restrict__ active, int *__restrict__ info, float *__restrict__ errs, float *__restrict__ Yout, float *__restrict__ Cout,
    double *__restrict__ yvec, const float *__restrict__ Tw, const float *__restrict__ Ys, int chunk) {
    __shared__ double red[UPD_THREADS / 64 + 1];
    extern __shared__ __attribute__((aligned(16))) char usmem[];
    const int part = (int)blockIdx.x >= D.B ? 1 : 0;
    const int b = (int)blockIdx.x - part * D.B;
    const int N = D.N, d = D.d, K = D.K, NN = N * N, Nd = N * d;
    const int tid = threadIdx.x;
    int *flag_out = active + (outer & 1) * 2 * D.B + part * D.B + b;
    if (!fgw_active(active, D.B, b, outer)) {
        if (tid == 0) *flag_out = 0;
        return;
    }
    constexpr int U = 4;
    double e2 = 0.0;
    if (part == 0) {
        if (!prm.fixed_features) {
            double *Yb = Yw + (size_t)b * Nd;
            if constexpr (Y_FROM_T) {
                float *Tl = reinterpret_cast<float *>(usmem), *Zl = Tl + (size_t)chunk * NN;
                const int lane = tid & 63, wave = __builtin_amdgcn_readfirstlane(tid >> 6), li = lane & 15, lk = lane >> 4;
                const int Mq = (N + 15) >> 4, Nq = (d + 15) >> 4;
                constexpr int NWU = UPD_THREADS / 64, TW = 2;
                for (int t0 = 0; t0 < Mq * Nq; t0 += NWU * TW) {
                    int ti0[TW], tj0[TW], tic[TW], tjc[TW];
                    bool mine[TW];
                    f64x4 sum[TW];
#pragma unroll
                    for (int w = 0; w < TW; ++w) {
                        const int t = t0 + wave + w * NWU;
                        mine[w] = t < Mq * Nq;
                        ti0[w] = mine[w] ? (t / Nq) << 4 : 0; tj0[w] = mine[w] ? (t % Nq) << 4 : 0;
                        tic[w] = min(ti0[w] + li, N - 1); tjc[w] = min(tj0[w] + li, d - 1);
                        sum[w] = f64x4{0.0, 0.0, 0.0, 0.0};
                    }
                    for (int s0 = 0; s0 < K; s0 += chunk) {
                        const int cs = min(chunk, K - s0);
                        __syncthreads();
                        const float *tg = Tw + ((size_t)b * K + s0) * NN, *zg = Ys + ((size_t)b * K + s0) * Nd;
                        auto stage = [&](const float *__restrict__ src, float *dst, int n) {
                            constexpr int SB = 12;
                            for (int base = 0; base < n; base += SB * UPD_THREADS) {
                                float v[SB];
#pragma unroll
                                for (int u = 0; u < SB; ++u) { const int q = base + u * UPD_THREADS + tid; v[u] = src[q < n ? q : n - 1]; }
#pragma unroll
                                for (int u = 0; u < SB; ++u) { const int q = base + u * UPD_THREADS + tid; if (q < n) dst[q] = v[u]; }
                            }
                        };
                        stage(tg, Tl, cs * NN);
                        stage(zg, Zl, cs * Nd);
                        __syncthreads();
#pragma unroll
                        for (int w = 0; w < TW; ++w)
                            if (mine[w])
                                for (int q = 0; q < cs; ++q) {
                                    const double lam = lambdas ? (double)lambdas[s0 + q] : 1.0 / (double)K;
                                    const f64x4 r = mm2_tile<0, false>(Tl + (size_t)q * NN + tic[w] * N + lk, Zl + (size_t)q * Nd + lk * d + tjc[w], d, N, lk);
                                    sum[w] = sum[w] + lam * r;
                                }
                    }
#pragma unroll
                    for (int w = 0; w < TW; ++w) {
                        const int jb = tj0[w] + li;
                        if (mine[w] && jb < d) {
#pragma unroll
                            for (int qq = 0; qq < 4; ++qq) {
                                const int i = ti0[w] + lk + 4 * qq;
                                if (i < N) {
                                    const double pw = pb ? (double)pb[(size_t)b * N + i] : 1.0 / (double)N;
                                    const double yn = sum[w][qq] * (pw > 0.0 ? 1.0 / pw : 0.0);
                                    const double df = yn - Yb[i * d + jb];
                                    e2 += df * df;
                                    Yb[i * d + jb] = yn;
                                    Yout[(size_t)b * Nd + i * d + jb] = (float)yn;
                                }
                            }
                        }
                    }
                }
            } else {
                for (int t0 = tid; t0 < Nd; t0 += U * UPD_THREADS) {
                    double acc[U], old[U];
#pragma unroll
                    for (int u = 0; u < U; ++u) {
                        const int t = t0 + u * UPD_THREADS;
                        acc[u] = 0.0; old[u] = 0.0;
                        if (t < Nd) {
                            old[u] = Yb[t];
                            for (int s = 0; s < K; ++s) {
                                const double lam = lambdas ? (double)lambdas[s] : 1.0 / (double)K;
                                const int i = t / d;
                                const double pw = pb ? (double)pb[(size_t)b * N + i] : 1.0 / (double)N;
                                const double pinv = pw > 0.0 ? 1.0 / pw : 0.0;
                                acc[u] += lam * Ypart[((size_t)b * K + s) * Nd + t] * pinv;
                            }
                        }
                    }
#pragma unroll
                    for (int u = 0; u < U; ++u) {
                        const int t = t0 + u * UPD_THREADS;
                        if (t < Nd) {
                            const double df = acc[u] - old[u];
                            e2 += df * df;
                            Yb[t] = acc[u];
                            Yout[(size_t)b * Nd + t] = (float)acc[u];
                        }
                    }
                }
            }
        }
    } else if (!prm.fixed_structure) {
        double *Cb = Cw + (size_t)b * NN;
        for (int t0 = tid; t0 < NN; t0 += U * UPD_THREADS) {
            double acc[U], old[U];
#pragma unroll
            for (int u = 0; u < U; ++u) {
                const int t = t0 + u * UPD_THREADS;
                acc[u] = 0.0; old[u] = 0.0;
                if (t < NN) {
                    old[u] = Cb[t];
                    for (int s = 0; s < K; ++s) {
                        const double lam = lambdas ? (double)lambdas[s] : 1.0 / (double)K;
                        acc[u] += lam * Cpart[((size_t)b * K + s) * NN + t];
                    }
                }
            }
#pragma unroll
            for (int u = 0; u < U; ++u) {
                const int t = t0 + u * UPD_THREADS;
                if (t < NN) {
                    const int i = t / N, j = t - i * N;
                    const double pi = pb ? (double)pb[(size_t)b * N + i] : 1.0 / (double)N;
                    const double pj = pb ? (double)pb[(size_t)b * N + j] : 1.0 / (double)N;
                    const double cn = pi * pj > 0.0 ? (prm.loss_fun ? exp(acc[u] / (pi * pj)) : acc[u] / (pi * pj)) : 0.0;
                    const double df = cn - old[u];
                    e2 += df * df;
                    Cb[t] = cn;
                    Cout[(size_t)b * NN + t] = (float)cn;
                }
            }
        }
    }
    const double err = sqrt(block_sum_d<UPD_THREADS / 64>(e2, red));
    if (yvec) molecule_vectors<UPD_THREADS>(Yw + (size_t)b * Nd, Cw + (size_t)b * NN, pb ? pb + (size_t)b * N : nullptr, N, d, prm.loss_fun != 0,
                                            yvec + (size_t)b * 2 * N, part);
    if (tid == 0) {
        errs[((size_t)b * 2 + part) * prm.max_iter + outer] = (float)err;
        info[b * 4 + 0] = outer + 1;
        *flag_out = err > (double)prm.tol ? 1 : 0;
    }
}

inline size_t small_lds(int N, int d) {
    const size_t NP = (size_t)N * fgw_pitch(N);
    (void)d; return NP * 8 * 4 + (256 + 128 + 8 + (NP >= (size_t)SK_SCRATCH_DOUBLES ? 0 : SK_SCRATCH_DOUBLES)) * 8 + NP * 4 * 2;
}

}

bool conan_fgw_small_supported(int N, int d) { return N <= 64 && small_lds(N, d) <= 160 * 1024; }

void conan_fgw_small_prepare(const FgwCall &c) {
    k_fgw_small_vectors<<<c.D.B * c.D.K, 256, 0, c.s>>>(c.Ys, c.Cs, c.ps, c.p, c.D, c.prm.loss_fun, c.Cw, c.Yw, c.zvec, c.yvec, c.init_C, c.init_Y,
                                                       c.prm.max_iter, c.active, c.info, c.errs, c.Y, c.C, c.adj);
}

template <class F>
static void with_rows(int R, F &&f) {
    if (R <= 6) f(std::integral_constant<int, 6>{});
    else if (R <= 9) f(std::integral_constant<int, 9>{});
    else if (R <= 12) f(std::integral_constant<int, 12>{});
    else f(std::integral_constant<int, 16>{});
}

template <int R, typename C2T>
static void launch_fast(const FgwCall &c, int outer, int y_zero, fgw_part_t *Ypart) {
    const FgwDims &D = c.D;
    const int tpw = fast_tiles_per_wave(D.N);
    auto go = [&](auto kernel) {
        launch_lds(kernel, D.B * D.K, FGW_THREADS, fast_lds<C2T>(D.N).bytes, c.s, c.Ys, c.Cs, c.ps, c.p, D, c.prm, fast_const(c.prm, D.N), outer,
                   y_zero, c.Cw, c.Yw, c.active, c.T, c.info, Ypart, c.Cpart, c.zvec, c.yvec, c.redo, c.adj);
    };
    if constexpr (R <= 6) go(k_fgw_coupling_fast<R, 1, C2T>);
    else if constexpr (R <= 12) { if (tpw <= 1) go(k_fgw_coupling_fast<R, 1, C2T>); else go(k_fgw_coupling_fast<R, 3, C2T>); }
    else { if (tpw <= 1) go(k_fgw_coupling_fast<R, 1, C2T>); else if (tpw <= 3) go(k_fgw_coupling_fast<R, 3, C2T>); else go(k_fgw_coupling_fast<R, 4, C2T>); }
}

bool conan_fgw_fast_supported(int N, int d, int small_int) {
    if (N > 64 || N < 4) return false;
    const size_t lds = small_int ? fast_lds<unsigned char>(N).bytes : fast_lds<float>(N).bytes;
    return lds <= 160 * 1024 && d >= 1;
}

void conan_fgw_small_coupling(const FgwCall &c, int outer, int y_zero, fgw_part_t *Ypart) {
    const FgwDims &D = c.D;
    const size_t lds = small_lds(D.N, D.d);
    const int grid = D.B * D.K;
    const bool kl = c.prm.loss_fun != 0;
    with_rows((D.N + 3) / 4, [&](auto R) {
        const int *only = nullptr;
        if (!kl && conan_fgw_fast_supported(D.N, D.d, c.prm.cs_small_int)) {
            if (c.prm.cs_small_int) launch_fast<R.value, unsigned char>(c, outer, y_zero, Ypart);
            else launch_fast<R.value, float>(c, outer, y_zero, Ypart);
            only = c.redo;
        }
        auto exact = [&](auto kernel, int blocks) {
            launch_lds(kernel, blocks, FGW_THREADS, lds, c.s, c.Ys, c.Cs, c.ps, c.p, D, c.prm, outer, y_zero, c.Cw, c.Yw, c.active, c.T, c.info, Ypart,
                       c.Cpart, c.zvec, c.yvec, only, c.adj);
        };
        if (kl) exact(k_fgw_coupling_small<R.value, true, false>, grid);
        else if (only) exact(k_fgw_coupling_small<R.value, false, true>, (grid + 63) / 64);
        else exact(k_fgw_coupling_small<R.value, false, false>, grid);
    });
}

void conan_fgw_small_update(const FgwCall &c, int outer, bool y_from_t) {
    const FgwDims &D = c.D;
    const int chunk = y_from_t ? conan_fgw_update_chunk(D.K, D.N, D.d, D.B) : 0;
    if (chunk > 0)
        launch_lds(k_fgw_update_parts<true>, 2 * D.B, UPD_THREADS, (size_t)chunk * ((size_t)D.N * D.N + (size_t)D.N * D.d) * 4, c.s, c.p, c.lambdas, D,
                   c.prm, outer, nullptr, c.Cpart, c.Cw, c.Yw, c.active, c.info, c.errs, c.Y, c.C, c.yvec, c.T, c.Ys, chunk);
    else
        k_fgw_update_parts<false><<<2 * D.B, UPD_THREADS, 0, c.s>>>(c.p, c.lambdas, D, c.prm, outer, c.Ypart, c.Cpart, c.Cw, c.Yw, c.active, c.info, c.errs,
                                                                     c.Y, c.C, c.yvec, nullptr, nullptr, 0);
}

int conan_fgw_update_chunk(int K, int N, int d, int B) {
    if (N > 64) return 0;
    const size_t per = ((size_t)N * N + (size_t)N * d) * 4, budget = (2 * B <= 256 ? 144 : 72) * 1024;
    if (per > budget) return 0;
    const int c = (int)(budget / per);
    return c < K ? c : K;
}
```

### conan-fgw_amd/ops.py

```python
from __future__ import annotations

import ctypes
import math
from typing import Optional

import torch
from torch import Tensor

from . import wgrad
from ._lib import FgwParams, call, lib, ptr, stream_ptr

f32, i32, i64 = torch.float32, torch.int32, torch.int64


def _c(t: Tensor) -> Tensor:
    return t if t.is_contiguous() else t.contiguous()


FUSED_GRAPH_BUILD = True


class RadiusGraph:

    def __init__(self, pos: Tensor, graph_ptr: Tensor, num_graphs: int, cutoff: float, max_num_neighbors: int, loop: bool = False,
# ... 585 lines not shown
            ctx.gmax = torch.empty(1, dtype=f32, device=x.device)
        call("conan_cfconv_fwd", ptr(x, f32), ptr(W, f32), ptr(graph.rowptr), ptr(graph.col), ptr(pid), graph.num_atoms, F,
             ptr(out), ptr(ctx.gmax), stream_ptr())
        ctx.graph, ctx.pre, ctx.pairs = graph, pre_cutoff_grad, use_pairs
        ctx.save_for_backward(x, W)
        return out

    @staticmethod
    def backward(ctx, dout):
        x, W = ctx.saved_tensors
        g = ctx.graph
        dout = _c(dout)
        dx = dW = None
        F = x.shape[1]
        if ctx.gmax is not None and ctx.needs_input_grad[0] and ctx.needs_input_grad[1]:
            t_rowptr, t_eid = g.transpose()
            dx = torch.empty_like(x)
            dW = torch.empty_like(W)
            call("conan_cfconv_bwd_xw_pairs", ptr(W), ptr(x), ptr(dout), ptr(t_rowptr), ptr(t_eid), ptr(g.tgt), ptr(g.pid), ptr(g.pair_e0), ptr(g.pair_e1),
                 ptr(g.pair_dist), float(g.cutoff), g.num_atoms, F, ptr(dx), ptr(dW), ptr(ctx.gmax), stream_ptr())
            _tag_gmax(dW, ctx.gmax)
            return dx, dW, None, None, None
        want_gmax = ctx.needs_input_grad[1] and ctx.pairs and F == 128
        gmax = torch.empty(1, dtype=f32, device=x.device) if want_gmax else None
        if ctx.needs_input_grad[0]:
            t_rowptr, t_eid = g.transpose()
            dx = torch.empty_like(x)
            call("conan_cfconv_bwd_x", ptr(W), ptr(dout), ptr(t_rowptr), ptr(t_eid), ptr(g.tgt), ptr(g.pid) if ctx.pairs else None,
                 g.num_atoms, F, ptr(dx), ptr(gmax), stream_ptr())
        elif gmax is not None:
            gmax.zero_()
        if ctx.needs_input_grad[1]:
            dW = torch.empty_like(W)
            if ctx.pairs:
                if not ctx.pre:
                    raise RuntimeError("use_pairs requires pre_cutoff_grad=True (the pair gradient includes the cosine cutoff)")
                call("conan_cfconv_bwd_w_pairs", ptr(x), ptr(dout), ptr(g.num_pairs_dev), g.max_edges, ptr(g.pair_e0), ptr(g.pair_e1), ptr(g.col),
                     ptr(g.tgt), F, ptr(g.pair_dist), float(g.cutoff), ptr(dW), ptr(gmax), stream_ptr())
                if gmax is not None:
                    _tag_gmax(dW, gmax)
            else:
                call("conan_cfconv_bwd_w", ptr(x), ptr(dout), ptr(g.num_edges_dev), g.max_edges, ptr(g.col), ptr(g.tgt), F,
                     ptr(g.dist) if ctx.pre else None, float(g.cutoff or 0.0), ptr(dW), stream_ptr())
        return dx, dW, None, None, None


def cfconv(x: Tensor, W: Tensor, graph: RadiusGraph, pre_cutoff_grad: bool = False, use_pairs: bool = False) -> Tensor:
    return _CFConvFn.apply(x, W, graph, pre_cutoff_grad, use_pairs)


class _SegmentSumFn(torch.autograd.Function):
    @staticmethod
    def forward(ctx, x, graph_ptr, num_graphs):
        x = _c(x)
        out = torch.empty(num_graphs, x.shape[1], dtype=f32, device=x.device)
        call("conan_segment_sum_fwd", ptr(x, f32), ptr(graph_ptr, i32), num_graphs, x.shape[1], ptr(out), stream_ptr())
        ctx.save_for_backward(graph_ptr)
        ctx.shape, ctx.G = x.shape, num_graphs
        return out

    @staticmethod
    def backward(ctx, dout):
        (gp,) = ctx.saved_tensors
        dx = torch.empty(ctx.shape, dtype=f32, device=dout.device)
        call("conan_segment_sum_bwd", ptr(_c(dout)), ptr(gp), ctx.G, ctx.shape[1], ptr(dx), stream_ptr())
        return dx, None, None


def segment_sum(x: Tensor, graph_ptr: Tensor, num_graphs: int) -> Tensor:
    return _SegmentSumFn.apply(x, graph_ptr, num_graphs)


class _DensifyFn(torch.autograd.Function):
    @staticmethod
    def forward(ctx, feat, graph, N, shift, a, b, adjacency=True):
        feat = _c(feat)
        G, d = graph.num_graphs, feat.shape[1]
        dev = feat.device
        Ys = torch.empty(G, N, d, dtype=f32, device=dev)
        Cs = torch.empty(G, N, N, dtype=f32, device=dev) if adjacency else torch.empty(0, dtype=f32, device=dev)
        minmax = torch.empty(G, 2, dtype=f32, device=dev)
        call("conan_fgw_densify", ptr(feat, f32), ptr(graph.graph_ptr), ptr(graph.rowptr), ptr(graph.col), G, N, d, shift, a, b,
             ptr(Ys), ptr(Cs) if adjacency else None, ptr(minmax), stream_ptr())
        ctx.save_for_backward(feat, minmax)
        ctx.graph, ctx.args = graph, (N, shift, a, b)
        ctx.mark_non_differentiable(Cs)
        ctx.set_materialize_grads(False)
        return Ys, Cs

    @staticmethod
    def backward(ctx, dYs, _dCs):
        if dYs is None:
            return None, None, None, None, None, None, None
        feat, minmax = ctx.saved_tensors
        N, shift, a, b = ctx.args
        g = ctx.graph
        dfeat = torch.empty_like(feat)
        call("conan_fgw_densify_bwd", ptr(feat), ptr(_c(dYs)), ptr(g.graph_ptr), ptr(minmax), g.num_graphs, N, feat.shape[1],
             shift, a, b, ptr(dfeat), stream_ptr())
        return dfeat, None, None, None, None, None, None


def fgw_densify(feat: Tensor, graph: RadiusGraph, max_nodes: int, shift: float, a: float = 0.1, b: float = 2.0, adjacency: bool = True):
    return _DensifyFn.apply(feat, graph, max_nodes, float(shift), float(a), float(b), bool(adjacency))


PROD_FGW = dict(alpha=0.1, epsilon=0.1, max_iter=5, tol=1e-2, inner_tol=1e-4, num_iter_max=5, stop_thr=1e-2,
                fixed_structure=False, fixed_features=False, warmstart=True)


FGW_SOLVERS = {"PGD": 0, "PPA": 1, "BAPG": 2}
_LOSS_CODE = {"square_loss": 0, "kl_loss": 1}


def _symmetric_code(symmetric) -> int:
    if symmetric is True:
        return 1
    if symmetric is False:
        return 0
    if symmetric is None:
        return -1
    raise ValueError(f"symmetric must be True, False or None, not {symmetric!r}")


def _fgw_params(alpha, epsilon, max_iter, tol, inner_tol, num_iter_max, stop_thr, fixed_structure, fixed_features, warmstart, loss_fun,
                cs_small_int=False) -> FgwParams:
    return FgwParams(float(alpha), float(epsilon), int(max_iter), float(tol), float(inner_tol), int(num_iter_max), float(stop_thr),
                     int(bool(fixed_structure)), int(bool(fixed_features)), int(bool(warmstart)), _LOSS_CODE[loss_fun], int(bool(cs_small_int)))


class _FgwBarycenterFn(torch.autograd.Function):
    @staticmethod
    def forward(ctx, Ys, Cs, ps, p, lambdas, init_C, init_Y, params):
        adj = params.get("adjacency")
        Ys = _c(Ys)
        Cs = _c(Cs) if adj is None else None
        B, K, N, d = Ys.shape
        if adj is not None and adj.num_graphs != B * K:
            raise RuntimeError(f"adjacency graph holds {adj.num_graphs} conformer graphs, Ys holds {B} x {K}")
        dev = Ys.device
        prm = _fgw_params(params["alpha"], params["epsilon"], params["max_iter"], params["tol"], params["inner_tol"], params["num_iter_max"],
                          params["stop_thr"], params["fixed_structure"], params["fixed_features"], params["warmstart"],
                          params.get("loss_fun", "square_loss"), params.get("cs_small_int", False))
        Y = torch.empty(B, N, d, dtype=f32, device=dev)
        C = torch.empty(B, N, N, dtype=f32, device=dev)
        T = torch.empty(B, K, N, N, dtype=f32, device=dev)
        T_iter = torch.empty(prm.max_iter, B, K, N, N, dtype=f32, device=dev) if params.get("keep_iterates") else None
        info = torch.empty(B, 4, dtype=i32, device=dev)
        errs = torch.empty(B, 2, prm.max_iter, dtype=f32, device=dev)
        solver = FGW_SOLVERS[params.get("solver", "PGD")]
        symmetric = _symmetric_code(params.get("symmetric", True))
        ws_bytes = lib().conan_fgw_workspace_bytes(B, K, N, d, int(adj is not None), solver, symmetric)
        ws = torch.empty(int(ws_bytes), dtype=torch.uint8, device=dev)
        common = (ptr(ps), ptr(p), ptr(lambdas), ptr(init_C), ptr(init_Y), B, K, N, d, ctypes.byref(prm), solver, symmetric,
                  ptr(Y), ptr(C), ptr(T), ptr(T_iter), ptr(info), ptr(errs), ptr(ws), stream_ptr())
        if adj is None:
            call("conan_fgw_barycenter_fwd", ptr(Ys, f32), ptr(Cs, f32), *common)
        else:
            call("conan_fgw_barycenter_fwd_ragged", ptr(Ys, f32), ptr(adj.graph_ptr, i32), ptr(adj.rowptr, i32), ptr(adj.col, i32), ptr(adj.tgt, i32),
                 *common)
        ctx.dims = (B, K, N, d)
        ctx.set_materialize_grads(False)
        need = ctx.needs_input_grad
        fs, ff = bool(params["fixed_structure"]), bool(params["fixed_features"])
        want = dict(Ys=need[0] and not ff, Cs=need[1] and Cs is not None and not fs, p=need[3] and p is not None,
                    lam=need[4] and lambdas is not None, init_C=need[5] and fs, init_Y=need[6] and ff)
        ctx.full = any(want[k] for k in ("Cs", "p", "lam", "init_C", "init_Y")) or (need[0] and ff)
        c_diff = want["init_C"] if fs else (want["Cs"] or want["p"] or want["lam"])
        if not ctx.full:
            ctx.save_for_backward(T, p, lambdas)
        else:
            kl = prm.loss_fun == 1
            ctx.want, ctx.flags = want, (prm.loss_fun, int(fs), int(ff))
            keep_Ys = want["lam"] and not ff
            keep_Cs = (want["Cs"] or want["lam"]) and not fs
            keep_Y = want["p"] and not ff
            keep_C = not fs and (want["p"] or (kl and (want["Cs"] or want["lam"])))
            ctx.save_for_backward(T, p, lambdas, Ys if keep_Ys else None, Cs if keep_Cs else None, Y if keep_Y else None,
                                  C if keep_C else None)
        nd = (T, info, errs) if c_diff else (C, T, info, errs)
        if T_iter is None:
            ctx.mark_non_differentiable(*nd)
            return Y, C, T, info, errs
        ctx.mark_non_differentiable(*nd, T_iter)
        return Y, C, T, info, errs, T_iter

    @staticmethod
    def backward(ctx, dY, dC=None, *_):
        if not ctx.full:
            if dY is None:
                return (None,) * 8
            T, p, lambdas = ctx.saved_tensors
            B, K, N, d = ctx.dims
            dYs = torch.empty(B, K, N, d, dtype=f32, device=dY.device)
            call("conan_fgw_barycenter_bwd", ptr(T), ptr(_c(dY)), ptr(p), ptr(lambdas), B, K, N, d, ptr(dYs), stream_ptr())
            return dYs, None, None, None, None, None, None, None
        if dY is None and dC is None:
            return (None,) * 8
        T, p, lambdas, Ys, Cs, Y, C = ctx.saved_tensors
        B, K, N, d = ctx.dims
        w = ctx.want
        loss, fs, ff = ctx.flags
        dev = T.device
        new = lambda want, *shape: torch.empty(*shape, dtype=f32, device=dev) if want else None
        dYs, dCs = new(w["Ys"], B, K, N, d), new(w["Cs"], B, K, N, N)
        dp = torch.empty_like(p) if w["p"] else None
        dlam = torch.empty_like(lambdas) if w["lam"] else None
        dinit_C, dinit_Y = new(w["init_C"], B, N, N), new(w["init_Y"], B, N, d)
        ws = torch.empty(int(lib().conan_fgw_barycenter_bwd_full_workspace_bytes(B, K, N, d)), dtype=torch.uint8, device=dev)
        opt = lambda t: ptr(_c(t)) if t is not None else None
        call("conan_fgw_barycenter_bwd_full", ptr(T), ptr(Ys), ptr(Cs), ptr(Y), ptr(C), opt(dY), opt(dC), ptr(p), ptr(lambdas), B, K, N, d,
             loss, fs, ff, ptr(dYs), ptr(dCs), ptr(dp), ptr(dlam), ptr(dinit_C), ptr(dinit_Y), ptr(ws), stream_ptr())
        return dYs, dCs, None, dp, dlam, dinit_C, dinit_Y, None


def fgw_barycenter_batched(Ys: Tensor, Cs: Tensor, ps: Optional[Tensor] = None, p: Optional[Tensor] = None,
                           lambdas: Optional[Tensor] = None, init_C: Optional[Tensor] = None, init_Y: Optional[Tensor] = None,
                           **params):
    if params.get("solver", "PGD") not in FGW_SOLVERS:
        raise ValueError("Unknown solver '%s'. Pick one in ['PGD', 'PPA', 'BAPG']." % params["solver"])
    _symmetric_code(params.get("symmetric", True))
    prm = dict(PROD_FGW)
    prm.update(params)
    opt = lambda t: _c(t) if t is not None else None
    return _FgwBarycenterFn.apply(Ys, Cs, opt(ps), opt(p), opt(lambdas), opt(init_C), opt(init_Y), prm)


def _pair_params(alpha, epsilon, max_iter, tol, num_iter_max, stop_thr, loss_fun, solver, symmetric):
    if solver not in FGW_SOLVERS:
        raise ValueError("Unknown solver '%s'. Pick one in ['PGD', 'PPA', 'BAPG']." % solver)
    if loss_fun not in ("square_loss", "kl_loss"):
        raise ValueError(f"Unknown `loss_fun='{loss_fun}'`. Use one of: {'square_loss', 'kl_loss'}.")
    prm = _fgw_params(alpha, epsilon, max_iter, tol, tol, num_iter_max, stop_thr, True, True, False, loss_fun)
    return prm, FGW_SOLVERS[solver], _symmetric_code(None if symmetric is None else bool(symmetric))


def _pair_tensor(t, name, *shape, keep_graph=False):
    if not t.is_cuda:
        raise NotImplementedError(f"the pairwise FGW solve runs on the GPU only: {name} is a CPU tensor")
    if tuple(t.shape) != shape:
        raise ValueError(f"{name} must have shape {list(shape)}, not {list(t.shape)}")
    return _c((t if keep_graph else t.detach()).to(f32))


def _pair_prepare(M, C1, C2, p, q, G0, keep_graph=False):
    if M.dim() != 3:
        raise ValueError(f"M must be [B,n1,n2], not {list(M.shape)}")
    B, n1, n2 = M.shape
    kg = dict(keep_graph=keep_graph)
    M, C1, C2 = _pair_tensor(M, "M", B, n1, n2, **kg), _pair_tensor(C1, "C1", B, n1, n1, **kg), _pair_tensor(C2, "C2", B, n2, n2, **kg)
    p = None if p is None else _pair_tensor(p, "p", B, n1, **kg)
    q = None if q is None else _pair_tensor(q, "q", B, n2, **kg)
    G0 = None if G0 is None else _pair_tensor(G0, "G0", B, n1, n2)
    dev, N = M.device, max(n1, n2)
    if n1 != n2:
        def pad(t, *shape):
            out = torch.zeros(B, *shape, dtype=f32, device=dev)
            out[(slice(None),) + tuple(slice(0, k) for k in t.shape[1:])] = t
            return out
        p = pad(torch.full((B, n1), 1.0 / n1, dtype=f32, device=dev) if p is None else p, N)
        q = pad(torch.full((B, n2), 1.0 / n2, dtype=f32, device=dev) if q is None else q, N)
        M, C1, C2 = pad(M, N, N), pad(C1, N, N), pad(C2, N, N)
        G0 = None if G0 is None else pad(G0, N, N)
    return M, C1, C2, p, q, G0, (B, N, n1, n2)


def _pair_fwd(M, C1, C2, p, q, G0, B, N, prm, solver_code, sym_code, with_dist):
    dev = M.device
    T = torch.empty(B, N, N, dtype=f32, device=dev)
    dist = torch.empty(B, dtype=f32, device=dev) if with_dist else None
    info = torch.empty(B, 4, dtype=i32, device=dev)
    errs = torch.empty(B, (prm.max_iter + 9) // 10, dtype=f32, device=dev)
    ws = torch.empty(int(lib().conan_fgw_pair_workspace_bytes(B, N, solver_code, sym_code)), dtype=torch.uint8, device=dev)
    call("conan_fgw_pair_fwd", ptr(M, f32), ptr(C1, f32), ptr(C2, f32), ptr(p), ptr(q), ptr(G0), B, N, ctypes.byref(prm), solver_code, sym_code,
         ptr(T), ptr(dist), ptr(info), ptr(errs), ptr(ws), stream_ptr())
    return T, dist, info, errs


def fgw_pair_batched(M: Tensor, C1: Tensor, C2: Tensor, p: Optional[Tensor] = None, q: Optional[Tensor] = None, G0: Optional[Tensor] = None, *,
                     alpha: float = 0.5, epsilon: float = 0.1, max_iter: int = 100, tol: float = 1e-5, num_iter_max: int = 100,
                     stop_thr: float = 1e-5, loss_fun: str = "square_loss", solver: str = "PGD", symmetric=None, with_dist: bool = True):
    prm, solver_code, sym_code = _pair_params(alpha, epsilon, max_iter, tol, num_iter_max, stop_thr, loss_fun, solver, symmetric)
    M, C1, C2, p, q, G0, (B, N, n1, n2) = _pair_prepare(M, C1, C2, p, q, G0)
    T, dist, info, errs = _pair_fwd(M, C1, C2, p, q, G0, B, N, prm, solver_code, sym_code, with_dist)
    return (T if n1 == n2 else T[:, :n1, :n2]), dist, info, errs


def _pair_list_stack(Ms, C1s, C2s, ps, qs, G0s, keep_graph=False):
    B = len(Ms)
    if B == 0 or len(C1s) != B or len(C2s) != B:
        raise ValueError("Ms, C1s and C2s must be non-empty lists of the same length")
    for t in list(Ms) + list(C1s) + list(C2s):
        if not t.is_cuda:
            raise NotImplementedError("the pairwise FGW solve runs on the GPU only: got a CPU tensor")
    dev = Ms[0].device
    sizes = [tuple(int(k) for k in m.shape) for m in Ms]
    Np = max(max(s) for s in sizes)

    def stack(ts, cols, default=None, keep=keep_graph):
        out = torch.zeros(B, *([Np] * cols), dtype=f32, device=dev)
        for b in range(B):
            t = ts[b] if ts is not None and ts[b] is not None else default(b)
            out[(b,) + tuple(slice(0, k) for k in t.shape)] = (t if keep else t.detach()).to(f32)
        return out

    G0 = None
    if G0s is not None and any(g is not None for g in G0s):
        if any(g is None for g in G0s):
            raise ValueError("G0s must hold a start plan for every pair or for none")
        G0 = stack(G0s, 2, keep=False)
    return (stack(Ms, 2), stack(C1s, 2), stack(C2s, 2), stack(ps, 1, lambda b: torch.full((sizes[b][0],), 1.0 / sizes[b][0], device=dev)),
            stack(qs, 1, lambda b: torch.full((sizes[b][1],), 1.0 / sizes[b][1], device=dev)), G0, sizes)


def fgw_pair_list(Ms, C1s, C2s, ps=None, qs=None, G0s=None, **params):
    M, C1, C2, p, q, G0, sizes = _pair_list_stack(Ms, C1s, C2s, ps, qs, G0s)
    T, dist, info, errs = fgw_pair_batched(M, C1, C2, p, q, G0, **params)
    return [T[b, :n1, :n2] for b, (n1, n2) in enumerate(sizes)], dist, info, errs


def _mixup_tensor(t, name, *shape):
    if not t.is_cuda:
        raise NotImplementedError(f"the FGWMixup solve runs on the GPU only: {name} is a CPU tensor")
    if tuple(t.shape) != shape:
        raise ValueError(f"{name} must have shape {list(shape)}, not {list(t.shape)}")
    return _c(t.detach().to(f32))


def _mixup_step(rho, epoch, eps):
    rho, epoch, eps = float(rho), int(epoch), float(eps)
    if not (rho > 0 and math.isfinite(rho)):
        raise ValueError(f"rho must be positive and finite, not {rho}")
    if epoch <= 0:
        raise ValueError(f"epoch must be positive, not {epoch}")
    return rho, epoch, eps


def fgw_acc_pair_batched(M: Tensor, A: Tensor, Bm: Tensor, a: Optional[Tensor] = None, b: Optional[Tensor] = None, X0: Optional[Tensor] = None, *,
                         alpha: float, rho: float, epoch: int = 200, eps: float = 1e-5, n1: Optional[Tensor] = None, n2: Optional[Tensor] = None):
    rho, epoch, eps = _mixup_step(rho, epoch, eps)
    if M.dim() != 3:
        raise ValueError(f"M must be [B,N1,N2], not {list(M.shape)}")
    B, N1, N2 = M.shape
    M, A, Bm = _mixup_tensor(M, "M", B, N1, N2), _mixup_tensor(A, "A", B, N1, N1), _mixup_tensor(Bm, "Bm", B, N2, N2)
    a = None if a is None else _mixup_tensor(a, "a", B, N1)
    b = None if b is None else _mixup_tensor(b, "b", B, N2)
    X0 = None if X0 is None else _mixup_tensor(X0, "X0", B, N1, N2)
    dev, N = M.device, max(N1, N2)
    if N1 != N2 or n1 is not None or n2 is not None:
        def own(n, Nc):
            n = torch.full((B,), Nc, device=dev) if n is None else torch.as_tensor(n, device=dev).reshape(B)
            return (torch.arange(N, device=dev)[None, :] < n[:, None]).to(f32), n.to(f32)

        def pad(t, *shape):
            out = torch.zeros(B, *shape, dtype=f32, device=dev)
            out[(slice(None),) + tuple(slice(0, k) for k in t.shape[1:])] = t
            return out
        (m1, c1), (m2, c2) = own(n1, N1), own(n2, N2)
        a = m1 / c1[:, None] if a is None else pad(a, N) * m1
        b = m2 / c2[:, None] if b is None else pad(b, N) * m2
        M, A, Bm = pad(M, N, N), pad(A, N, N), pad(Bm, N, N)
        X0 = None if X0 is None else pad(X0, N, N)
    X = torch.empty(B, N, N, dtype=f32, device=dev)
    objs = torch.empty(B, (epoch + 9) // 10, dtype=f32, device=dev)
    info = torch.empty(B, 4, dtype=i32, device=dev)
    ws = torch.empty(int(lib().conan_fgw_acc_pair_workspace_bytes(B, N)), dtype=torch.uint8, device=dev)
    call("conan_fgw_acc_pair_fwd", ptr(M, f32), ptr(A, f32), ptr(Bm, f32), ptr(a), ptr(b), ptr(X0), B, N, float(alpha), rho, epoch, eps,
         ptr(X), ptr(objs), ptr(info), ptr(ws), stream_ptr())
# ... 294 lines not shown
```

### conan-fgw_amd/schnet.py

```python
from __future__ import annotations

import math
from typing import Callable, Optional

import torch
from torch import Tensor
from torch.nn import Embedding, Linear, ModuleList, Sequential

from . import ops

OptTensor = Optional[Tensor]


class ShiftedSoftplus(torch.nn.Module):

    def __init__(self):
        super().__init__()
        self.shift = math.log(2.0)

    def forward(self, x: Tensor) -> Tensor:
        return ops.shifted_softplus(x)


class GaussianSmearing(torch.nn.Module):
# ... 40 lines not shown
        self.nn = nn
        self.cutoff = cutoff
        self.reset_parameters()

    def reset_parameters(self):
        torch.nn.init.xavier_uniform_(self.lin1.weight)
        torch.nn.init.xavier_uniform_(self.lin2.weight)
        self.lin2.bias.data.fill_(0)

    def forward(self, x: Tensor, graph: ops.RadiusGraph, rbf, tap: bool = False):
        if isinstance(rbf, Tensor):
            md = graph.num_edges_dev
            h1 = ops.linear(rbf, self.nn[0].weight, self.nn[0].bias, act=True, m_dev=md)
            w_raw = ops.linear(h1, self.nn[2].weight, self.nn[2].bias, m_dev=md)
            W = ops.cutoff_scale(w_raw, graph)
        else:
            offset, coeff = rbf
            if (FUSE_FILTER_INTO_GATHER and not torch.is_grad_enabled() and _filter_tensor_outgrows_cache(graph, self.nn[2].weight.shape[0])
                    and ops.filter_cfconv_supported(offset.shape[0], self.nn[2].weight.shape[0])):
                x_in = x if tap else None
                x = ops.linear(x, self.lin1.weight)
                x = ops.filter_cfconv(x, graph, offset, coeff, self.nn[0].weight, self.nn[0].bias, self.nn[2].weight, self.nn[2].bias)
                return (x, x_in) if tap else x
            W = ops.filter_generate(graph, offset, coeff, self.nn[0].weight, self.nn[0].bias, self.nn[2].weight, self.nn[2].bias)
        x_in = None
        if tap:
            x, x_in = ops.linear_tap(x, self.lin1.weight)
        else:
            x = ops.linear(x, self.lin1.weight)
        fused = not isinstance(rbf, Tensor)
        x = ops.cfconv(x, W, graph, pre_cutoff_grad=fused, use_pairs=fused)
        return (x, x_in) if tap else x


class InteractionBlock(torch.nn.Module):
    def __init__(self, hidden_channels: int, num_gaussians: int, num_filters: int, cutoff: float):
        super().__init__()
        self.mlp = Sequential(Linear(num_gaussians, num_filters), ShiftedSoftplus(), Linear(num_filters, num_filters))
        self.conv = CFConv(hidden_channels, hidden_channels, num_filters, self.mlp, cutoff)
        self.act = ShiftedSoftplus()
        self.lin = Linear(hidden_channels, hidden_channels)
        self.reset_parameters()

    def reset_parameters(self):
        torch.nn.init.xavier_uniform_(self.mlp[0].weight)
        self.mlp[0].bias.data.fill_(0)
        torch.nn.init.xavier_uniform_(self.mlp[2].weight)
        self.mlp[2].bias.data.fill_(0)
        self.conv.reset_parameters()
        torch.nn.init.xavier_uniform_(self.lin.weight)
        self.lin.bias.data.fill_(0)

    def forward(self, x: Tensor, graph: ops.RadiusGraph, rbf: Tensor) -> Tensor:
        m, x = self.conv(x, graph, rbf, tap=True)
        return ops.mlp2(m, self.conv.lin2.weight, self.conv.lin2.bias, self.lin.weight, self.lin.bias, residual=x)


class SchNetNoSum(torch.nn.Module):
    FEATURE_SHIFT = 0.5
    READOUT_MODE = 0

    def __init__(self, device, hidden_channels: int = 128, num_filters: int = 128, num_interactions: int = 6,
                 num_gaussians: int = 50, cutoff: float = 10.0, interaction_graph: Optional[Callable] = None,
                 max_num_neighbors: int = 32, readout: str = "add", dipole: bool = False, mean: Optional[float] = None,
                 std: Optional[float] = None, atomref: OptTensor = None, use_covalent: bool = False, use_readout: bool = True):
        super().__init__()
        if interaction_graph is not None:
            raise NotImplementedError("custom interaction_graph callables are not supported; the radius graph is a HIP kernel")
        if use_covalent:
            raise NotImplementedError("use_covalent=True (ESAN-only branch, schnet_no_sum.py:132-142) is out of scope")
        if dipole or atomref is not None:
            raise NotImplementedError("dipole / atomref are not used by ConAN (common.py:524-529)")
        if readout not in ("add", "sum"):
            raise NotImplementedError("only the sum readout is used by ConAN")
        self.device = device
        self.hidden_channels = hidden_channels
        self.num_filters = num_filters
        self.num_interactions = num_interactions
        self.num_gaussians = num_gaussians
        self.cutoff = cutoff
        self.use_readout = use_readout
        self.use_covalent = use_covalent
        self.fused_filter = True
        self.mean, self.std, self.scale = mean, std, None
        self.embedding = Embedding(100, hidden_channels, padding_idx=0)
        self.interaction_graph = RadiusInteractionGraph(cutoff, max_num_neighbors)
        self.distance_expansion = GaussianSmearing(0.0, cutoff, num_gaussians)
        self.interactions = ModuleList([InteractionBlock(hidden_channels, num_gaussians, num_filters, cutoff)
                                        for _ in range(num_interactions)])
        self.lin1 = Linear(hidden_channels, hidden_channels // 2)
        self.act = ShiftedSoftplus()
        self.register_buffer("initial_atomref", None)
        self.atomref = None
        torch.nn.init.xavier_uniform_(self.lin1.weight)
        self.lin1.bias.data.fill_(0)
        self.lin1_bary = Linear(hidden_channels, hidden_channels // 2)
        self.lin2_bary = Linear(hidden_channels // 2, hidden_channels // 2)
        self.lin2 = Linear(hidden_channels // 2, hidden_channels // 2)

    def _graphs(self, z: Tensor, pos: Tensor, batch: OptTensor, num_graphs: Optional[int]):
        if not z.is_cuda:
            raise RuntimeError("SchNetNoSum (MI355X) runs on the GPU only: move the inputs to the device; there is no CPU fallback")
        batch = torch.zeros_like(z) if batch is None else batch
        hint_g, hint_n = ops.batch_hints(batch)
        if num_graphs is None:
            num_graphs = hint_g if hint_g is not None else int(batch[-1].item()) + 1
        gptr = ops.graph_ptr_from_batch(batch, num_graphs)
        pairs = self.fused_filter and ops.filter_fused_supported(self.num_gaussians, self.num_filters)
        graph = self.interaction_graph.csr(pos, gptr, num_graphs, pairs=pairs, transpose=torch.is_grad_enabled())
        graph.max_nodes_hint = hint_n if hint_g == num_graphs else None
        return batch, gptr, graph, num_graphs

    def _trunk(self, z: Tensor, graph: ops.RadiusGraph) -> Tensor:
        h = ops.embedding(z, self.embedding.weight, self.embedding.padding_idx)
        if self.fused_filter and ops.filter_fused_supported(self.num_gaussians, self.num_filters):
            rbf = (self.distance_expansion.offset, self.distance_expansion.coeff)
        else:
            rbf = self.distance_expansion(graph)
        for interaction in self.interactions:
            h = interaction(h, graph, rbf)
        return h

    def _head(self, h: Tensor, lin1: Linear, lin2: Linear) -> Tensor:
        return ops.mlp2_outact(h, lin1.weight, lin1.bias, lin2.weight, lin2.bias)

    def forward(self, z: Tensor, pos: Tensor, batch: OptTensor = None, data_batch=None, num_graphs: Optional[int] = None) -> Tensor:
        batch, gptr, graph, G = self._graphs(z, pos, batch, num_graphs)
        h = self._head(self._trunk(z, graph), self.lin1, self.lin2)
        return ops.segment_sum(h, gptr, G) if self.use_readout else h

    def forward_3d_bary(self, z: Tensor, pos: Tensor, batch: OptTensor = None, data_batch=None, num_graphs: Optional[int] = None,
                        _graph=None):
        if _graph is None:
            _, _, graph, _ = self._graphs(z, pos, batch, num_graphs)
        else:
            graph = _graph
        h_shared = self._trunk(z, graph)
        return ops.mlp2_outact_dual(h_shared, *((l1.weight, l1.bias, l2.weight, l2.bias)
                                                for l1, l2 in ((self.lin1, self.lin2), (self.lin1_bary, self.lin2_bary))))

    def _solve_barycenter(self, node_feature: Tensor, edge_index, batch: Tensor, batch_size: int, num_conformers: int,
                          max_nodes: Optional[int] = None):
        K = num_conformers
        G = batch_size * K
        if isinstance(edge_index, ops.RadiusGraph):
            graph = edge_index
        else:
            graph = _graph_from_edge_index(edge_index, batch, G)
        if max_nodes is None:
            max_nodes = getattr(graph, "max_nodes_hint", None)
        if max_nodes is None:
            gp = graph.graph_ptr
            max_nodes = int((gp[1:] - gp[:-1]).max().item())
        Ys, _ = ops.fgw_densify(node_feature, graph, max_nodes, self.FEATURE_SHIFT, adjacency=False)
        N, d = max_nodes, node_feature.shape[1]
        Y, C, T, info, errs = ops.fgw_barycenter_batched(Ys.view(batch_size, K, N, d), None, adjacency=graph)
        self.last_fgw = dict(Y=Y, C=C, T=T, info=info, errs=errs, Ys=Ys)
        return Y, graph

    def _compute_barycenter(self, node_feature: Tensor, edge_index, batch: Tensor, batch_size: int, num_conformers: int,
                            max_nodes: Optional[int] = None, _want_node_out: bool = True):
        Y, graph = self._solve_barycenter(node_feature, edge_index, batch, batch_size, num_conformers, max_nodes)
        F_bary_batch = ops.fgw_readout(Y, num_conformers, self.READOUT_MODE)
        node_out = ops.segment_sum(node_feature, graph.graph_ptr, batch_size * num_conformers) if _want_node_out else None
        return node_out, F_bary_batch

    def forward_w_barycenter_parts(self, z: Tensor, pos: Tensor, num_conformers: int, batch: OptTensor = None, num_graphs: Optional[int] = None,
                                   max_nodes: Optional[int] = None):
        batch, gptr, graph, G = self._graphs(z, pos, batch, num_graphs)
        h_3d, h_bary = self.forward_3d_bary(z, pos, batch, _graph=graph)
        Y, _ = self._solve_barycenter(h_bary, graph, batch, G // num_conformers, num_conformers, max_nodes=max_nodes)
        return h_3d, gptr, Y

    def forward_w_barycenter(self, z: Tensor, pos: Tensor, num_conformers: int, batch: OptTensor = None, data_batch=None,
                             max_iter: int = 100, epsilon: float = 0.1, num_graphs: Optional[int] = None,
                             max_nodes: Optional[int] = None):
        h_3d, gptr, Y = self.forward_w_barycenter_parts(z, pos, num_conformers, batch, num_graphs=num_graphs, max_nodes=max_nodes)
        h_bary = ops.fgw_readout(Y, num_conformers, self.READOUT_MODE)
        h_3d = ops.segment_sum(h_3d, gptr, gptr.numel() - 1)
        return h_3d, h_bary


def _graph_from_edge_index(edge_index: Tensor, batch: Tensor, num_graphs: int) -> ops.RadiusGraph:
    g = object.__new__(ops.RadiusGraph)
    n = batch.shape[0]
    src, tgt = edge_index[0], edge_index[1]
    order = torch.argsort(tgt * n + src)
    src, tgt = src[order], tgt[order]
    deg = torch.bincount(tgt, minlength=n)
    rowptr = torch.zeros(n + 1, dtype=torch.int32, device=batch.device)
    rowptr[1:] = deg.cumsum(0).to(torch.int32)
    g.num_atoms, g.num_graphs = n, num_graphs
    g.graph_ptr = ops.graph_ptr_from_batch(batch, num_graphs)
    g.rowptr, g.col, g.tgt = rowptr, src.to(torch.int32).contiguous(), tgt.to(torch.int32).contiguous()
    g.dist = None
    g.max_edges = max(1, int(src.shape[0]))
    g.num_edges_dev = rowptr[n:]
    g._num_edges = int(src.shape[0])
    g._t_rowptr = g._t_eid = None
    g.pid = None
    g._deg = torch.empty(n + 1, dtype=torch.int32, device=batch.device)
    g.cutoff = g.cap = g.loop = None
    return g
```

### include/conan_fgw_hip.h

```cpp
#ifndef CONAN_FGW_HIP_H
#define CONAN_FGW_HIP_H

#include <stdint.h>

#ifdef __cplusplus
extern "C" {
#endif

#define CONAN_OK 0
#define CONAN_E_BADARG (-1)
#define CONAN_E_LAUNCH (-2)
#define CONAN_E_UNSUPPORTED (-3)

#define CONAN_FGW_ABI_VERSION 6
int conan_abi_version(void);


typedef struct conan_batch_layout {
    int B, K;
    int num_graphs;
    int num_atoms;
    int num_bond_edges;
    int max_nodes;
    int x_dim, ea_dim;
// ... 115 lines not shown
                               const int *graph_ptr, float agg_weight, int num_molecules, int K, int N, int D, int readout_mode, float *dh3, float *dxc,
                               float *dY, float *dW3, float *db3, float *dWb, float *dbb, float *dwreg, float *dbreg, void *stream);

int conan_mse_loss_fwd(const float *pred, const float *target, int n, float *loss, float *dpred, void *stream);

int conan_bce_loss_fwd(const float *pred, const float *target, const float *weight, int n_weight, int n, float *loss, float *dpred, void *stream);

int conan_adam_flat_step(float *params, const float *grads, float *exp_avg, float *exp_avg_sq, float *step_dev, unsigned *ticket_dev, long long n,
                         double lr, double beta1, double beta2, double eps, double weight_decay, const double *lr_dev, void *stream);

#define CONAN_GRAD_CLIP_MAX_BLOCKS 256
int conan_grad_clip_flat(float *grads, long long n, double max_norm, float *norm_coef_dev, double *partials_dev, unsigned *ticket_dev, void *stream);

int conan_mlp2_supported(int M, int K, int N1, int N2);
int conan_mlp2_fwd(const float *x, const float *w1, const float *b1, const float *w2, const float *b2, const float *residual, int M, int K, int N1,
                   int N2, float *mid_out, float *y, void *stream);
int conan_mlp2_bwd(const float *dy, const float *w2, const float *w1, const float *mid, int M, int K, int N1, int N2, float *dmid_out, float *dx,
                   void *stream);
int conan_mlp2_outact_supported(int M, int K, int N1, int N2);
int conan_mlp2_outact_fwd(const float *x, const float *w1, const float *b1, const float *w2, const float *b2, int M, int K, int N1, int N2,
                          float *mid_out, float *y, void *stream);
int conan_mlp2_outact_bwd(const float *dy, const float *y, const float *w2, const float *w1, int M, int K, int N1, int N2, float *g_out,
                          float *dmid_out, float *dx, void *stream);
int conan_mlp2_outact_dual_fwd(const float *x, const float *w1a, const float *b1a, const float *w2a, const float *b2a, const float *w1b, const float *b1b,
                               const float *w2b, const float *b2b, int M, int K, int N1, int N2, const int *m_dev, int form, float *mid_a, float *y_a,
                               float *mid_b, float *y_b, void *stream);
int conan_mlp2_outact_dual_bwd(const float *dy_a, const float *y_a, const float *w2a, const float *w1a, const float *dy_b, const float *y_b,
                               const float *w2b, const float *w1b, int M, int K, int N1, int N2, const int *m_dev, float *g_a, float *dmid_a, float *g_b,
                               float *dmid_b, float *dx, void *stream);

int conan_filter_fused_supported(int num_gaussians, int num_filters);
int conan_filter_fwd(const float *dist, const int *num_edges_dev, int max_edges, const float *offset, int num_gaussians,
                     float coeff, float cutoff, int num_filters, const float *w1, const float *b1, const float *w2,
                     const float *b2, float *W, float *h1_out, void *stream);

int conan_filter_cfconv_fwd_supported(int num_gaussians, int num_filters);
int conan_filter_cfconv_fwd(const float *x, const float *dist, const int *col, const int *tgt, const int *num_edges_dev, int max_edges,
                            const float *offset, int num_gaussians, float coeff, float cutoff, int num_filters, const float *w1,
                            const float *b1, const float *w2, const float *b2, int num_atoms, float *out, void *stream);

int conan_cfconv_fwd(const float *x, const float *W, const int *rowptr, const int *col, const int *pid, int num_atoms,
                     int num_filters, float *out, float *zero_slot, void *stream);
int conan_cfconv_bwd_x(const float *W, const float *dout, const int *t_rowptr, const int *t_eid, const int *tgt,
                       const int *pid, int num_atoms, int num_filters, float *dx, float *zero_slot, void *stream);
int conan_cfconv_bwd_w_pairs(const float *x, const float *dout, const int *num_pairs_dev, int max_pairs, const int *pair_e0,
                             const int *pair_e1, const int *col, const int *tgt, int num_filters, const float *pair_dist,
                             float cutoff, float *dWp, float *gmax, void *stream);
int conan_cfconv_bwd_xw_pairs_supported(int num_filters);
int conan_cfconv_bwd_xw_pairs(const float *W, const float *x, const float *dout, const int *t_rowptr, const int *t_eid, const int *tgt, const int *pid,
                              const int *pair_e0, const int *pair_e1, const float *pair_dist, float cutoff, int num_atoms, int num_filters, float *dx,
                              float *dWp, float *gmax, void *stream);
int conan_cfconv_bwd_w(const float *x, const float *dout, const int *num_edges_dev, int max_edges, const int *col,
                       const int *tgt, int num_filters, const float *dist, float cutoff, float *dW, void *stream);

int conan_segment_sum_fwd(const float *x, const int *graph_ptr, int num_graphs, int width, float *out, void *stream);
int conan_segment_sum_bwd(const float *dout, const int *graph_ptr, int num_graphs, int width, float *dx, void *stream);


int conan_visnet_edge_unit(const float *pos, const int *col, const int *tgt, const int *num_edges_dev, int max_edges,
                           float *dvec, void *stream);
int conan_visnet_expnormal(const float *dist, const int *num_edges_dev, int max_edges, const float *means,
                           const float *betas, int num_rbf, float alpha, float cutoff, float *out, void *stream);
int conan_visnet_neighbor_scale(float *W, const float *dist, const int *col, const int *tgt, const int *num_edges_dev,
                                int max_edges, int H, float cutoff, void *stream);
int conan_visnet_neighbor_scale_to(const float *W, const float *dist, const int *col, const int *tgt, const int *num_edges_dev,
                                   int max_edges, int H, float cutoff, float *out, void *stream);
int conan_concat2(const float *a, int Ha, const float *b, int Hb, long long rows, float *out, void *stream);
int conan_visnet_edge_embed(const float *x, const float *p, const int *col, const int *tgt, const int *num_edges_dev,
                            int max_edges, int H, float *f, void *stream);
int conan_layernorm_fwd(const float *x, const float *gamma, const float *beta, int rows, int H, float eps, float *out,
                        void *stream);
int conan_scale_channels(const float *v, const float *w, long long rows, int H, float *out, void *stream);
int conan_scale_channels_add(const float *v, const float *w, const float *add, long long rows, int H, float *out, void *stream);
int conan_visnet_vecdot(const float *vp, int n, int H, float *out, void *stream);
int conan_visnet_attn_message(const float *q, const float *k, const float *v, const float *dk, const float *dv,
                              const int *rowptr, const int *col, const float *dist, float cutoff, int n, int H,
                              int num_heads, int pre_act, float *vmsg, float *xagg, void *stream);
int conan_visnet_vec_aggregate(const float *vec, const float *s, const float *dvec, const int *rowptr, const int *col,
                               int n, int H, int pre_act, float *vagg, void *stream);
int conan_visnet_node_update(const float *x, const float *vec, const float *vdot, const float *o, const float *vp,
                             const float *vagg, int n, int H, float *x_out, float *vec_out, void *stream);
int conan_visnet_edge_update(const float *wt, const float *ws, const float *t, const float *dvec, const int *col,
                             const int *tgt, const int *num_edges_dev, int max_edges, int H, int pre_act, const float *f,
                             float *f_out, void *stream);
int conan_visnet_spatial_norm(const float *v, int n, int H, float *out, void *stream);
int conan_visnet_gate(const float *u, const float *v2, int n, int out_channels, int scalar_activation, float *x_out,
                      float *v_out, void *stream);
int conan_visnet_prior(const float *x, const int64_t *z, const float *atomref, const float *std_dev, int n,
                       int out_channels, float *out, void *stream);

int conan_silu_fwd(const float *x, int rows, int width, const int *m_dev, float *y, void *stream);
int conan_silu_bwd(const float *x, const float *dy, int rows, int width, const int *m_dev, float *dx, void *stream);
int conan_split2(const float *in, int Ha, int Hb, long long rows, float *a, float *b, void *stream);
int conan_rowsum(const float *x, int rows, int width, float *out, void *stream);
int conan_scale_scalar(const float *x, const float *scale_dev, long long count, float *out, void *stream);
int conan_visnet_edge_embed_bwd(const float *x, const float *p, const float *df, const int *rowptr, const int *col,
                                const int *tgt, const int *t_rowptr, const int *t_eid, const int *num_edges_dev,
                                int max_edges, int n, int H, float *dp, float *dx, void *stream);
long long conan_layernorm_bwd_ws(int rows, int H);
int conan_layernorm_bwd(const float *x, const float *gamma, const float *dy, int rows, int H, float eps, float *dx,
                        float *dgamma, float *dbeta, float *ws, void *stream);
int conan_layernorm_bwd_res(const float *x, const float *gamma, const float *dy, const float *dres, int rows, int H, float eps, float *dx,
                            float *dgamma, float *dbeta, float *ws, void *stream);
int conan_visnet_vecdot_bwd(const float *vp, const float *dout, int n, int H, float *dvp, void *stream);
int conan_visnet_attn_message_bwd(const float *q, const float *k, const float *v, const float *dk, const float *dv,
                                  const float *dvmsg, const float *dxagg, const int *rowptr, const int *col,
                                  const int *tgt, const int *t_rowptr, const int *t_eid, const float *dist, float cutoff,
                                  int n, int H, int num_heads, int pre_act, float *dq, float *dkn, float *dvn, float *ddk,
                                  float *ddv, void *stream);
int conan_visnet_vec_aggregate_bwd(const float *vec, const float *s, const float *dvec3, const float *dvagg,
                                   const int *col, const int *tgt, const int *t_rowptr, const int *t_eid,
                                   const int *num_edges_dev, int max_edges, int n, int H, int pre_act, float *ds,
                                   float *dvec, void *stream);
int conan_visnet_node_update_bwd(const float *dxo, const float *dveco, const float *vdot, const float *o, const float *vp,
                                 int n, int H, float *dvdot, float *dout_o, float *dvp, void *stream);
int conan_visnet_edge_update_bwd(const float *wt, const float *ws, const float *t, const float *dvec3, const float *dfo,
                                 const int *rowptr, const int *col, const int *tgt, const int *t_rowptr, const int *t_eid,
                                 int n, int H, int pre_act, float *dwt, float *dws, float *dt, void *stream);
int conan_visnet_spatial_norm_bwd(const float *v, const float *dout, int n, int H, float *dv, void *stream);
int conan_visnet_gate_bwd(const float *u, const float *v2, const float *dxo, const float *dvo, int n, int out_channels,
                          int scalar_activation, float *du, float *dv2, void *stream);


int conan_fgw_densify(const float *feat, const int *graph_ptr, const int *rowptr, const int *col, int num_graphs,
                      int N, int d, float shift, float a, float b, float *Ys, float *Cs, float *minmax, void *stream);
int conan_fgw_densify_bwd(const float *feat, const float *dYs, const int *graph_ptr, const float *minmax,
                          int num_graphs, int N, int d, float shift, float a, float b, float *dfeat, void *stream);

typedef struct conan_fgw_params {
    float alpha;
    float epsilon;
    int max_iter;
    float tol;
    float inner_tol;
    int num_iter_max;
    float stop_thr;
    int fixed_structure;
    int fixed_features;
    int warmstart;
    int loss_fun;
    int cs_small_int;
} conan_fgw_params;

long long conan_fgw_workspace_bytes(int B, int K, int N, int d, int ragged, int solver, int symmetric);
int conan_fgw_barycenter_fwd(const float *Ys, const float *Cs, const float *ps, const float *p, const float *lambdas,
                             const float *init_C, const float *init_Y, int B, int K, int N, int d,
                             const conan_fgw_params *params , int solver, int symmetric, float *Y, float *C, float *T,
                             float *T_iter, int *info, float *errs, void *workspace, void *stream);
int conan_fgw_barycenter_fwd_ragged(const float *Ys, const int *graph_ptr, const int *rowptr, const int *col, const int *tgt, const float *ps,
                                    const float *p, const float *lambdas, const float *init_C, const float *init_Y, int B, int K, int N, int d,
                                    const conan_fgw_params *params , int solver, int symmetric, float *Y, float *C, float *T,
                                    float *T_iter, int *info, float *errs, void *workspace, void *stream);

long long conan_fgw_pair_workspace_bytes(int B, int N, int solver, int symmetric);
int conan_fgw_pair_fwd(const float *M, const float *C1, const float *C2, const float *p, const float *q, const float *G0, int B, int N,
                       const conan_fgw_params *params , int solver, int symmetric, float *T, float *fgw_dist, int *info,
                       float *errs, void *workspace, void *stream);
int conan_fgw_pair_dist(const float *M, const float *C1, const float *C2, const float *p, const float *q, const float *T, int B, int N,
                        float alpha, int loss_fun, float *out, void *stream);
int conan_fgw_pair_dist_bwd(const float *C1, const float *C2, const float *p, const float *q, const float *T, const float *gout,
                            int B, int N, float alpha, int loss_fun,
                            float *dM, float *dC1, float *dC2, float *dp, float *dq, void *stream);

int conan_fgw_acc_lds_resident(int N);
long long conan_fgw_acc_pair_workspace_bytes(int B, int N);
int conan_fgw_acc_pair_fwd(const float *M, const float *A, const float *Bm, const float *a, const float *b, const float *X0, int B, int N,
                           double alpha, double rho, int epoch, double eps, float *X, float *objs, int *info, void *workspace, void *stream);
long long conan_fgw_mixup_workspace_bytes(int B, int K, int N, int d);
int conan_fgw_mixup_barycenter_fwd(const float *Ys, const float *Cs, const float *ps, const float *p, const float *lambdas,
                                   const float *init_C, const float *init_Y, int B, int K, int N, int d,
                                   const conan_fgw_params *params , double rho, int epoch, double eps, float *Y, float *C, float *T,
                                   float *T_iter, int *info, float *errs, void *workspace, void *stream);

long long conan_sinkhorn_workspace_bytes(int B, int N1, int N2);
int conan_sinkhorn_lds_resident(int n1, int n2);
int conan_sinkhorn_fwd(const float *M, const float *a, const float *b, const float *warm_u, const float *warm_v, const int *n1, const int *n2,
                       int B, int N1, int N2, long long m_batch_stride, float reg, int method, int num_iter_max, float stop_thr, float *T,
                       float *loss, float *log_u, float *log_v, int *info, float *errs, void *workspace, void *stream);

int conan_fgw_barycenter_bwd(const float *T, const float *dY, const float *p, const float *lambdas, int B, int K,
                             int N, int d, float *dYs, void *stream);

long long conan_fgw_barycenter_bwd_full_workspace_bytes(int B, int K, int N, int d);
int conan_fgw_barycenter_bwd_full(const float *T, const float *Ys, const float *Cs, const float *Y, const float *C, const float *dY,
                                  const float *dC, const float *p, const float *lambdas, int B, int K, int N, int d, int loss_fun,
                                  int fixed_structure, int fixed_features, float *dYs, float *dCs, float *dp, float *dlambdas,
                                  float *dinit_C, float *dinit_Y, void *workspace, void *stream);

int conan_fgw_readout_fwd(const float *Y, int B, int K, int N, int d, int mode, float *out, void *stream);
int conan_fgw_readout_bwd(const float *Y, const float *dout, int B, int K, int N, int d, int mode, float *dY,
                          void *stream);

int conan_unary_fwd(const float *x, long long count, int op, float *y, void *stream);
int conan_unary_bwd(const float *y, const float *dy, long long count, int op, float *dx, void *stream);

int conan_zero_tail(float *buf, const int *m_dev, int rows, int width, void *stream);


int conan_bond_graph_csr(const int64_t *edge_index, int num_edges, int num_nodes, int *ws, int *rowptr, int *col, int *eid,
                         int *t_rowptr, int *t_pos, int *t_tgt, void *stream);
int conan_gat_edge_vec(const float *w_edge, const float *att_edge, int channels, int edge_dim, float *v, void *stream);
int conan_gat_edge_vec_bwd(const float *w_edge, const float *att_edge, const float *dv, int channels, int edge_dim,
                           float *dw_edge, float *datt_edge, void *stream);
int conan_gat_node_alpha(const float *h, const float *att_src, const float *att_dst, int n, int channels, float *a_src,
                         float *a_dst, void *stream);
int conan_gat_aggregate_fwd(const float *h, const float *a_src, const float *a_dst, const int *rowptr, const int *col,
                            const int *eid, const float *edge_attr, int edge_dim, const float *v, const float *bias,
                            float negative_slope, int n, int channels, float *out, float *alpha, float *alpha_self, void *stream);
long long conan_gat_bwd_ws(int n, int num_edges, int channels, int edge_dim);
int conan_gat_aggregate_bwd(const float *h, const float *dout, const float *alpha, const float *alpha_self, const float *a_src,
                            const float *a_dst, const float *att_src, const float *att_dst, const int *rowptr, const int *col,
                            const int *eid, const int *t_rowptr, const int *t_pos, const int *t_tgt, const float *edge_attr,
                            int edge_dim, const float *v, float negative_slope, int n, int num_edges, int channels, float *ws,
                            float *dh, float *dparams, void *stream);

#ifdef __cplusplus
}
#endif
#endif
```

Before: 116,300.

## Fuse feature densify into FGW small-path prologue and backward into one kernel

Feature densification (per-graph min/max normalisation into dense Ys) is deferred and done inside the small-solver vectors prologue kernel, which removes a separate launch and a global round trip. The backward barycenter gradient and densify backward are merged into one LDS-resident kernel, so the dYs intermediate is no longer materialised. The size-bucket base computation in fgw_order_by_size becomes a wave-level parallel prefix scan instead of a serial loop on one thread. This adds thread-local pending state between the Python calls and a more complex API surface.

```diff
diff --git a/conan-fgw_amd/_lib.py b/conan-fgw_amd/_lib.py
--- a/conan-fgw_amd/_lib.py
+++ b/conan-fgw_amd/_lib.py
@@ -154,6 +154,11 @@
                                          _P, _P, _P, _P, _P, _P, _P, _P]),
     "conan_fgw_barycenter_fwd_ragged": (c_int, [_P, _P, _P, _P, _P, _P, _P, _P, _P, _P, c_int, c_int, c_int, c_int, ctypes.POINTER(FgwParams),
                                                 c_int, c_int, _P, _P, _P, _P, _P, _P, _P, _P]),
+    "conan_fgw_densify_deferred": (c_int, [_P, _P, c_int, c_int, c_int, c_float, c_float, c_float, _P, _P]),
+    "conan_fgw_feat_supported": (c_int, [c_int] * 5),
+    "conan_fgw_barycenter_prologue_ragged": (c_int, [_P] * 10 + [c_int, c_int, c_int, c_int, ctypes.POINTER(FgwParams), c_int, c_int] + [_P] * 8),
+    "conan_fgw_workspace_order_offset": (c_ll, [c_int] * 7),
+    "conan_fgw_set_order_scan": (c_int, [c_int]),
     "conan_fgw_pair_workspace_bytes": (c_ll, [c_int, c_int, c_int, c_int]),
     "conan_fgw_pair_fwd": (c_int, [_P, _P, _P, _P, _P, _P, c_int, c_int, ctypes.POINTER(FgwParams), c_int, c_int, _P, _P, _P, _P, _P, _P]),
     "conan_fgw_pair_dist": (c_int, [_P, _P, _P, _P, _P, _P, c_int, c_int, c_float, c_int, _P, _P]),
@@ -167,6 +172,7 @@
     "conan_sinkhorn_lds_resident": (c_int, [c_int, c_int]),
     "conan_sinkhorn_fwd": (c_int, [_P] * 7 + [c_int, c_int, c_int, c_ll, c_float, c_int, c_int, c_float] + [_P] * 8),
     "conan_fgw_barycenter_bwd": (c_int, [_P, _P, _P, _P, c_int, c_int, c_int, c_int, _P, _P]),
+    "conan_fgw_barycenter_bwd_feat": (c_int, [_P, _P, _P, _P, c_int, c_int, c_int, c_int, _P, _P, _P, c_float, c_float, c_float, _P, _P]),
     "conan_fgw_barycenter_bwd_full_workspace_bytes": (c_ll, [c_int, c_int, c_int, c_int]),
     "conan_fgw_barycenter_bwd_full": (c_int, [_P, _P, _P, _P, _P, _P, _P, _P, _P, c_int, c_int, c_int, c_int, c_int, c_int, c_int,
                                               _P, _P, _P, _P, _P, _P, _P, _P]),
diff --git a/conan-fgw_amd/csrc/fgw.hip b/conan-fgw_amd/csrc/fgw.hip
--- a/conan-fgw_amd/csrc/fgw.hip
+++ b/conan-fgw_amd/csrc/fgw.hip
@@ -1,4 +1,5 @@
 #include "fgw_coupling.h"
+#include <atomic>
 #ifdef CONAN_FGW_PROFILE
 FGW_PROF_ACCESSOR(conan_debug_fgw_prof_large)
 FGW_PROF_TRACE_ACCESSOR(conan_debug_fgw_trace_large)
@@ -521,6 +522,61 @@
     for (int t = n * d + tid; t < n_raw * d; t += 256) dfeat[(size_t)lo * d + t] = __builtin_nanf("");
 }
 
+__global__ void __launch_bounds__(256) k_fgw_bwd_densify(const float *__restrict__ T, const float *__restrict__ dY, const float *__restrict__ pb,
+                                                         const float *__restrict__ lambdas, int K, int N, int d, const float *__restrict__ feat,
+                                                         const int *__restrict__ gptr, const float *__restrict__ minmax, float shift, float a,
+                                                         float b, float *__restrict__ dfeat) {
+    extern __shared__ float bw_smem[];
+    __shared__ float red[4], tot[4];
+    const int g = blockIdx.x, tid = threadIdx.x;
+    const int bm = g / K, sg = g % K;
+    const float *Ts = T + (size_t)g * N * N;
+    const float *gy = dY + (size_t)bm * N * d;
+    const float lam = lambdas ? lambdas[sg] : 1.0f / (float)K;
+    const int lo = gptr[g], n_raw = gptr[g + 1] - lo;
+    const int n = n_raw > N ? N : n_raw;
+    const float mn = minmax[g * 2], mx = minmax[g * 2 + 1];
+    const float s = b - a, r = mx - mn;
+    float *Tl = bw_smem, *gl = bw_smem + N * N, *G = gl + N * d;
+    for (int t = tid; t < N * N; t += 256) Tl[t] = Ts[t];
+    for (int t = tid; t < N * d; t += 256) {
+        const int i = t / d;
+        const float pinv = pb ? (pb[(size_t)bm * N + i] > 0.f ? 1.0f / pb[(size_t)bm * N + i] : 0.f) : (float)N;
+        gl[t] = pinv * gy[t];
+    }
+    __syncthreads();
+    float s0 = 0.f, s1 = 0.f, cmin = 0.f, cmax = 0.f;
+    for (int t = tid; t < N * d; t += 256) {
+        const int j = t / d, c = t - j * d;
+        const float x = (t < n * d ? feat[(size_t)lo * d + t] : 0.f) + shift;
+        float acc = 0.f;
+        for (int i = 0; i < N; ++i) acc += Tl[i * N + j] * gl[i * d + c];
+        float gg = lam * acc;
+        asm volatile("" : "+v"(gg));
+        G[t] = gg;
+        s0 += gg; s1 += gg * (x - mn);
+        cmin += (x == mn) ? 1.f : 0.f; cmax += (x == mx) ? 1.f : 0.f;
+    }
+    float vals[4] = {s0, s1, cmin, cmax};
+    for (int q = 0; q < 4; ++q) {
+        float v = wave_sum(vals[q]);
+        if ((tid & 63) == 0) red[tid >> 6] = v;
+        __syncthreads();
+        if (tid == 0) tot[q] = red[0] + red[1] + red[2] + red[3];
+        __syncthreads();
+    }
+    const float dmn = -tot[0] * s / r + tot[1] * s / (r * r);
+    const float dmx = -tot[1] * s / (r * r);
+    for (int t = tid; t < n * d; t += 256) {
+        const float x = feat[(size_t)lo * d + t] + shift;
+        float gx = G[t] * s / r;
+        if (x == mn) gx += dmn / tot[2];
+        if (x == mx) gx += dmx / tot[3];
+        dfeat[(size_t)lo * d + t] = gx;
+    }
+    for (int t = n * d + tid; t < n_raw * d; t += 256) dfeat[(size_t)lo * d + t] = __builtin_nanf("");
+}
+
 __global__ void __launch_bounds__(64) k_readout_fwd(const float *__restrict__ Y, int K, int N, int d, int mode, float *__restrict__ out) {
     const int b = blockIdx.x;
     const float *Yb = Y + (size_t)b * N * d;
@@ -604,6 +660,25 @@
     return w;
 }
 
+struct FgwFeat {
+    const float *feat;
+    float shift, a, b;
+    float *minmax;
+};
+inline bool fgw_feat_supported(int N, int d, int solver, int symmetric, int loss_fun) {
+    return solver == 0 && symmetric == 1 && loss_fun == 0 && N > 0 && d > 0 && conan_fgw_small_supported(N, d) && conan_fgw_fast_supported(N, d, 1);
+}
+struct FgwPending {
+    FgwFeat ft;
+    const int *gptr;
+    float *Ys;
+    int G, N, d;
+    bool valid;
+};
+thread_local FgwPending g_pending{};
+inline size_t bwd_densify_lds(int N, int d) { return ((size_t)N * N + 2 * (size_t)N * d) * sizeof(float); }
+std::atomic<int> g_order_scan{1};
+
 enum class FgwPath {
     Small,
     Big,
@@ -633,8 +708,10 @@
 
 int fgw_fwd_impl(const float *Ys, const float *Cs, const float *ps, const float *p, const float *lambdas, const float *init_C,
                  const float *init_Y, int B, int K, int N, int d, const conan_fgw_params *params, float *Y, float *C, float *T, float *T_iter,
-                 int *info, float *errs, void *workspace, void *stream, FgwAdj adj, int solver, int symmetric) {
+                 int *info, float *errs, void *workspace, void *stream, FgwAdj adj, int solver, int symmetric, const FgwFeat *ft = nullptr,
+                 bool prologue_only = false) {
     if (solver < 0 || solver > 2 || symmetric < -1 || symmetric > 1) return CONAN_E_BADARG;
+    if (ft && !(ft->feat && ft->minmax && params && fgw_feat_supported(N, d, solver, symmetric, params->loss_fun) && adj.rowptr)) return CONAN_E_BADARG;
     if (!Ys || !(Cs || (adj.gptr && adj.rowptr && adj.col && adj.tgt)) || !params || !Y || !C || !T || !info || !errs || !workspace || B <= 0 || K <= 0 || N <= 0 || d <= 0)
         return CONAN_E_BADARG;
     if (params->max_iter <= 0 || params->num_iter_max <= 0) return CONAN_E_BADARG;
@@ -656,6 +733,8 @@
     c.Ypart = ws_at<fgw_part_t>(workspace, w.Ypart); c.Cpart = ws_at<fgw_part_t>(workspace, w.Cpart);
     c.redo = ws_at<int>(workspace, w.redo);
     c.asym_scratch = ws_at<char>(workspace, w.asym);
+    c.order_scan = g_order_scan.load(std::memory_order_relaxed) != 0;
+    if (ft) { c.feat = ft->feat; c.shift = ft->shift; c.na = ft->a; c.nb = ft->b; c.Ys_out = const_cast<float *>(Ys); c.minmax = ft->minmax; }
     c.s = as_stream(stream);
     if (ragged) {
         c.prm.cs_small_int = 1;
@@ -683,6 +762,7 @@
 
     if (pl.path == FgwPath::Small) conan_fgw_small_prepare(c);
     else k_fgw_init<<<B, 256, 0, c.s>>>(c.Cs, init_C, init_Y, c.D, c.prm.max_iter, c.Cw, c.Yw, c.active, info, errs, Y, C, c.adj);
+    if (prologue_only) { CONAN_LAUNCH_CHECK(); return CONAN_OK; }
     const FastConst fc = fast_const(c.prm, N);
     for (int outer = 0; outer < c.prm.max_iter; ++outer) {
         const int y_zero = (outer == 0 && !init_Y) ? 1 : 0;
@@ -731,8 +811,59 @@
                                     const float *p, const float *lambdas, const float *init_C, const float *init_Y, int B, int K, int N, int d,
                                     const conan_fgw_params *params, int solver, int symmetric, float *Y, float *C, float *T, float *T_iter,
                                     int *info, float *errs, void *workspace, void *stream) {
+    const FgwPending pend = g_pending;
+    g_pending = FgwPending{};
+    if (pend.valid) {
+        if (pend.Ys != Ys || pend.gptr != graph_ptr || (long long)pend.G != (long long)B * K || pend.N != N || pend.d != d || !params || !rowptr || !col)
+            return CONAN_E_BADARG;
+        if (fgw_feat_supported(N, d, solver, symmetric, params->loss_fun))
+            return fgw_fwd_impl(Ys, nullptr, ps, p, lambdas, init_C, init_Y, B, K, N, d, params, Y, C, T, T_iter, info, errs, workspace, stream,
+                                FgwAdj{graph_ptr, rowptr, col, tgt, nullptr, nullptr}, solver, symmetric, &pend.ft);
+        k_densify<<<pend.G, 256, 0, as_stream(stream)>>>(pend.ft.feat, graph_ptr, rowptr, col, N, d, pend.ft.shift, pend.ft.a, pend.ft.b, pend.Ys, nullptr,
+                                                        pend.ft.minmax);
+    }
     return fgw_fwd_impl(Ys, nullptr, ps, p, lambdas, init_C, init_Y, B, K, N, d, params, Y, C, T, T_iter, info, errs, workspace, stream,
                         FgwAdj{graph_ptr, rowptr, col, tgt, nullptr, nullptr}, solver, symmetric);
+}
+
+int conan_fgw_densify_deferred(const float *feat, const int *graph_ptr, int num_graphs, int N, int d, float shift, float a, float b, float *Ys,
+                               float *minmax) {
+    g_pending = FgwPending{};
+    if (!feat || !graph_ptr || !Ys || !minmax || num_graphs <= 0 || N <= 0 || d <= 0) return CONAN_E_BADARG;
+    g_pending = FgwPending{FgwFeat{feat, shift, a, b, minmax}, graph_ptr, Ys, num_graphs, N, d, true};
+    return CONAN_OK;
+}
+
+int conan_fgw_feat_supported(int N, int d, int solver, int symmetric, int loss_fun) {
+    if (N <= 0 || d <= 0) return 0;
+    return (fgw_feat_supported(N, d, solver, symmetric, loss_fun) ? 1 : 0) | (bwd_densify_lds(N, d) <= 64 * 1024 ? 2 : 0);
+}
+
+int conan_fgw_barycenter_prologue_ragged(const float *Ys, const int *graph_ptr, const int *rowptr, const int *col, const int *tgt, const float *ps,
+                                         const float *p, const float *lambdas, const float *init_C, const float *init_Y, int B, int K, int N,
+                                         int d, const conan_fgw_params *params, int solver, int symmetric, float *Y, float *C, float *T,
+                                         float *T_iter, int *info, float *errs, void *workspace, void *stream) {
+    return fgw_fwd_impl(Ys, nullptr, ps, p, lambdas, init_C, init_Y, B, K, N, d, params, Y, C, T, T_iter, info, errs, workspace, stream,
+                        FgwAdj{graph_ptr, rowptr, col, tgt, nullptr, nullptr}, solver, symmetric, nullptr, true);
+}
+
+long long conan_fgw_workspace_order_offset(int B, int K, int N, int d, int ragged, int solver, int symmetric) {
+    if (ragged != 0 && ragged != 1) return -1;
+    const FgwWorkspace w = fgw_workspace(B, K, N, d, ragged != 0, solver, symmetric);
+    return w.total ? (long long)w.order : -1;
+}
+
+int conan_fgw_set_order_scan(int on) { return g_order_scan.exchange(on ? 1 : 0); }
+
+int conan_fgw_barycenter_bwd_feat(const float *T, const float *dY, const float *p, const float *lambdas, int B, int K, int N, int d,
+                                  const float *feat, const int *graph_ptr, const float *minmax, float shift, float a, float b, float *dfeat,
+                                  void *stream) {
+    if (!T || !dY || !feat || !graph_ptr || !minmax || !dfeat || B <= 0 || K <= 0 || N <= 0 || d <= 0) return CONAN_E_BADARG;
+    const size_t lds = bwd_densify_lds(N, d);
+    if (lds > 64 * 1024) return CONAN_E_BADARG;
+    k_fgw_bwd_densify<<<B * K, 256, lds, as_stream(stream)>>>(T, dY, p, lambdas, K, N, d, feat, graph_ptr, minmax, shift, a, b, dfeat);
+    CONAN_LAUNCH_CHECK();
+    return CONAN_OK;
 }
 
 int conan_fgw_barycenter_bwd(const float *T, const float *dY, const float *p, const float *lambdas, int B, int K,
diff --git a/conan-fgw_amd/csrc/fgw_common.h b/conan-fgw_amd/csrc/fgw_common.h
--- a/conan-fgw_amd/csrc/fgw_common.h
+++ b/conan-fgw_amd/csrc/fgw_common.h
@@ -275,7 +275,7 @@
 }
 
 template <int NT>
-__device__ __forceinline__ void fgw_order_by_size(const FgwAdj &adj, int B, int K, int tid) {
+__device__ __forceinline__ void fgw_order_by_size(const FgwAdj &adj, int B, int K, int tid, bool scan = false) {
     static_assert(NT >= 256, "one thread per size bin");
     __shared__ unsigned char nsz[4096];
     __shared__ int hist[256], base[256];
@@ -288,7 +288,21 @@
         atomicAdd(&hist[n], 1);
     }
     __syncthreads();
-    if (tid == 0) {
+    if (scan) {
+    if (tid < 64) {
+        const int v0 = 255 - 4 * tid;
+        const int h0 = hist[v0], h1 = hist[v0 - 1], h2 = hist[v0 - 2], h3 = hist[v0 - 3];
+        const int own = h0 + h1 + h2 + h3;
+        int incl = own;
+#pragma unroll
+        for (int o = 1; o < 64; o <<= 1) {
+            const int up = __shfl_up(incl, o, 64);
+            incl += tid >= o ? up : 0;
+        }
+        const int excl = incl - own;
+        base[v0] = excl; base[v0 - 1] = excl + h0; base[v0 - 2] = excl + h0 + h1; base[v0 - 3] = excl + h0 + h1 + h2;
+    }
+    } else if (tid == 0) {
         int run = 0;
         for (int v = 255; v >= 0; --v) { base[v] = run; run += hist[v]; }
     }
@@ -960,6 +974,10 @@
     fgw_part_t *Ypart, *Cpart;
     double *zvec, *yvec;
     int *redo;
+    const float *feat;
+    float shift, na, nb;
+    float *Ys_out, *minmax;
+    bool order_scan;
     char *asym_scratch;
     hipStream_t s;
 };
diff --git a/conan-fgw_amd/csrc/fgw_small.hip b/conan-fgw_amd/csrc/fgw_small.hip
--- a/conan-fgw_amd/csrc/fgw_small.hip
+++ b/conan-fgw_amd/csrc/fgw_small.hip
@@ -857,17 +857,50 @@
     if (i < N && sub == 0) { if (which != 1) out[i] = y2; if (which != 0) out[N + i] = r1; }
 }
 
+struct FgwDensify {
+    const float *feat;
+    float shift, a, b;
+    float *Ys, *minmax;
+};
+template <bool DENSIFY>
 __global__ void __launch_bounds__(256) k_fgw_small_vectors(const float *__restrict__ Ys, const float *__restrict__ Cs, const float *__restrict__ ps,
                                                            const float *__restrict__ pb, FgwDims D, int kl, double *__restrict__ Cw,
                                                            double *__restrict__ Yw, double *__restrict__ zvec, double *__restrict__ yvec,
                                                            const float *__restrict__ init_C, const float *__restrict__ init_Y, int max_iter,
                                                            int *__restrict__ active, int *__restrict__ info, float *__restrict__ errs,
-                                                           float *__restrict__ Yout, float *__restrict__ Cout, FgwAdj adj) {
+                                                           float *__restrict__ Yout, float *__restrict__ Cout, FgwAdj adj, FgwDensify dn,
+                                                           int order_scan) {
     const int b = blockIdx.x / D.K, s = blockIdx.x % D.K;
     const int N = D.N, d = D.d;
     __shared__ __attribute__((aligned(16))) unsigned char cm[64 * 65 + 16];
     const int Pm = D.P;
-    if (adj.rowptr) {
+    if constexpr (DENSIFY) {
+        __shared__ float smn[4], smx[4];
+        const int g = (int)blockIdx.x, tid = (int)threadIdx.x;
+        const int lo = adj.gptr[g], n_raw = adj.gptr[g + 1] - lo;
+        const bool overflow = n_raw > N;
+        const int n = overflow ? N : n_raw;
+        for (int t = tid; t < (64 * 65 + 16) / 4; t += 256) reinterpret_cast<unsigned *>(cm)[t] = 0u;
+        float mn = 3.0e38f, mx = -3.0e38f;
+        for (int t = tid; t < n * d; t += 256) { const float v = dn.feat[(size_t)lo * d + t] + dn.shift; mn = fminf(mn, v); mx = fmaxf(mx, v); }
+        if (n < N) { const float v = 0.f + dn.shift; mn = fminf(mn, v); mx = fmaxf(mx, v); }
+        mn = wave_min(mn); mx = wave_max(mx);
+        if ((tid & 63) == 0) { smn[tid >> 6] = mn; smx[tid >> 6] = mx; }
+        __syncthreads();
+        adj_scatter_lds_bytes<256>(adj, g, N, Pm, cm, tid);
+        mn = fminf(fminf(smn[0], smn[1]), fminf(smn[2], smn[3]));
+        mx = fmaxf(fmaxf(smx[0], smx[1]), fmaxf(smx[2], smx[3]));
+        if (overflow) mn = mx = __builtin_nanf("");
+        if (tid == 0) { dn.minmax[g * 2] = mn; dn.minmax[g * 2 + 1] = mx; }
+        const float scale = dn.b - dn.a, range = mx - mn;
+        float *Yg = dn.Ys + (size_t)g * N * d;
+        for (int t = tid; t < N * d; t += 256) {
+            const float x = (t < n * d ? dn.feat[(size_t)lo * d + t] : 0.f) + dn.shift;
+            Yg[t] = dn.a + __fdiv_rn((x - mn) * scale, range);
+        }
+        __threadfence_block();
+        __syncthreads();
+    } else if (adj.rowptr) {
         for (int t = threadIdx.x; t < (64 * 65 + 16) / 4; t += 256) reinterpret_cast<unsigned *>(cm)[t] = 0u;
         __syncthreads();
         adj_scatter_lds_bytes<256>(adj, (int)blockIdx.x, N, Pm, cm, (int)threadIdx.x);
@@ -888,7 +921,7 @@
         for (int t = threadIdx.x; t < 2 * max_iter; t += 256) errs[(size_t)b * 2 * max_iter + t] = __builtin_nanf("");
         __syncthreads();
     }
-    const float *Z = Ys + ((size_t)b * D.K + s) * N * d;
+    const float *Z = (DENSIFY ? dn.Ys : Ys) + ((size_t)b * D.K + s) * N * d;
     const float *C2 = Cs + ((size_t)b * D.K + s) * N * N;
     const float *q = ps ? ps + ((size_t)b * D.K + s) * N : nullptr;
     const int j = (int)threadIdx.x >> 2, sub = (int)threadIdx.x & 3;
@@ -906,7 +939,7 @@
     if (j < N && sub == 0) { zo[j] = z2; zo[N + j] = r2; }
     if (s == 0)
         molecule_vectors<256>(Yw + (size_t)b * N * d, Cw + (size_t)b * N * N, pb ? pb + (size_t)b * N : nullptr, N, d, kl != 0, yvec + (size_t)b * 2 * N);
-    if (adj.order && blockIdx.x == gridDim.x - 1) fgw_order_by_size<256>(adj, D.B, D.K, (int)threadIdx.x);
+    if (adj.order && blockIdx.x == gridDim.x - 1) fgw_order_by_size<256>(adj, D.B, D.K, (int)threadIdx.x, order_scan != 0);
 }
 
 constexpr int UPD_THREADS = 512;
@@ -1058,7 +1091,8 @@
         }
     }
     const double err = sqrt(block_sum_d<UPD_THREADS / 64>(e2, red));
-    if (yvec) molecule_vectors<UPD_THREADS>(Yw + (size_t)b * Nd, Cw + (size_t)b * NN, pb ? pb + (size_t)b * N : nullptr, N, d, prm.loss_fun != 0,
+    if (yvec && outer + 1 < prm.max_iter)
+        molecule_vectors<UPD_THREADS>(Yw + (size_t)b * Nd, Cw + (size_t)b * NN, pb ? pb + (size_t)b * N : nullptr, N, d, prm.loss_fun != 0,
                                             yvec + (size_t)b * 2 * N, part);
     if (tid == 0) {
         errs[((size_t)b * 2 + part) * prm.max_iter + outer] = (float)err;
@@ -1077,8 +1111,13 @@
 bool conan_fgw_small_supported(int N, int d) { return N <= 64 && small_lds(N, d) <= 160 * 1024; }
 
 void conan_fgw_small_prepare(const FgwCall &c) {
-    k_fgw_small_vectors<<<c.D.B * c.D.K, 256, 0, c.s>>>(c.Ys, c.Cs, c.ps, c.p, c.D, c.prm.loss_fun, c.Cw, c.Yw, c.zvec, c.yvec, c.init_C, c.init_Y,
-                                                       c.prm.max_iter, c.active, c.info, c.errs, c.Y, c.C, c.adj);
+    const FgwDensify dn{c.feat, c.shift, c.na, c.nb, c.Ys_out, c.minmax};
+    auto go = [&](auto kernel) {
+        kernel<<<c.D.B * c.D.K, 256, 0, c.s>>>(c.Ys, c.Cs, c.ps, c.p, c.D, c.prm.loss_fun, c.Cw, c.Yw, c.zvec, c.yvec, c.init_C, c.init_Y, c.prm.max_iter,
+                                               c.active, c.info, c.errs, c.Y, c.C, c.adj, dn, c.order_scan ? 1 : 0);
+    };
+    if (c.feat) go(k_fgw_small_vectors<true>);
+    else go(k_fgw_small_vectors<false>);
 }
 
 template <class F>
diff --git a/conan-fgw_amd/ops.py b/conan-fgw_amd/ops.py
--- a/conan-fgw_amd/ops.py
+++ b/conan-fgw_amd/ops.py
@@ -761,6 +761,7 @@
         symmetric = _symmetric_code(params.get("symmetric", True))
         ws_bytes = lib().conan_fgw_workspace_bytes(B, K, N, d, int(adj is not None), solver, symmetric)
         ws = torch.empty(int(ws_bytes), dtype=torch.uint8, device=dev)
+        lib().conan_fgw_set_order_scan(int(bool(FGW_ORDER_SCAN)))
         common = (ptr(ps), ptr(p), ptr(lambdas), ptr(init_C), ptr(init_Y), B, K, N, d, ctypes.byref(prm), solver, symmetric,
                   ptr(Y), ptr(C), ptr(T), ptr(T_iter), ptr(info), ptr(errs), ptr(ws), stream_ptr())
         if adj is None:
@@ -823,6 +824,77 @@
         return dYs, dCs, None, dp, dlam, dinit_C, dinit_Y, None
 
 
+FGW_FUSED_DENSIFY = True
+FGW_FUSED_BACKWARD = True
+FGW_ORDER_SCAN = True
+
+
+class _DensifyBarycenterFn(torch.autograd.Function):
+    @staticmethod
+    def forward(ctx, feat, graph, B, K, N, shift, a, b, params):
+        feat = _c(feat)
+        d = feat.shape[1]
+        can = lib().conan_fgw_feat_supported(N, d, 0, 1, 0)
+        dev = feat.device
+        G = B * K
+        if graph.num_graphs != G:
+            raise RuntimeError(f"adjacency graph holds {graph.num_graphs} conformer graphs, the batch holds {B} x {K}")
+        prm = _fgw_params(params["alpha"], params["epsilon"], params["max_iter"], params["tol"], params["inner_tol"], params["num_iter_max"],
+                          params["stop_thr"], params["fixed_structure"], params["fixed_features"], params["warmstart"], "square_loss")
+        Ys = torch.empty(G, N, d, dtype=f32, device=dev)
+        minmax = torch.empty(G, 2, dtype=f32, device=dev)
+        Y = torch.empty(B, N, d, dtype=f32, device=dev)
+        C = torch.empty(B, N, N, dtype=f32, device=dev)
+        T = torch.empty(B, K, N, N, dtype=f32, device=dev)
+        info = torch.empty(B, 4, dtype=i32, device=dev)
+        errs = torch.empty(B, 2, prm.max_iter, dtype=f32, device=dev)
+        ws = torch.empty(int(lib().conan_fgw_workspace_bytes(B, K, N, d, 1, 0, 1)), dtype=torch.uint8, device=dev)
+        lib().conan_fgw_set_order_scan(int(bool(FGW_ORDER_SCAN)))
+        lists = (ptr(graph.graph_ptr, i32), ptr(graph.rowptr, i32), ptr(graph.col, i32), ptr(graph.tgt, i32))
+        common = (None, None, None, None, None, B, K, N, d, ctypes.byref(prm), 0, 1, ptr(Y), ptr(C), ptr(T), None, ptr(info), ptr(errs), ptr(ws),
+                  stream_ptr())
+        if FGW_FUSED_DENSIFY and can & 1:
+            call("conan_fgw_densify_deferred", ptr(feat, f32), lists[0], G, N, d, shift, a, b, ptr(Ys), ptr(minmax))
+        else:
+            call("conan_fgw_densify", ptr(feat, f32), lists[0], lists[1], lists[2], G, N, d, shift, a, b, ptr(Ys), None, ptr(minmax), stream_ptr())
+        call("conan_fgw_barycenter_fwd_ragged", ptr(Ys, f32), *lists, *common)
+        ctx.save_for_backward(feat, minmax, T)
+        ctx.graph, ctx.args = graph, (B, K, N, d, shift, a, b, bool(can & 2))
+        ctx.mark_non_differentiable(C, T, info, errs, Ys, minmax)
+        ctx.set_materialize_grads(False)
+        return Y, C, T, info, errs, Ys, minmax
+
+    @staticmethod
+    def backward(ctx, dY, *_):
+        if dY is None:
+            return (None,) * 9
+        feat, minmax, T = ctx.saved_tensors
+        B, K, N, d, shift, a, b, can_bwd = ctx.args
+        g = ctx.graph
+        dfeat = torch.empty_like(feat)
+        if FGW_FUSED_BACKWARD and can_bwd:
+            call("conan_fgw_barycenter_bwd_feat", ptr(T), ptr(_c(dY)), None, None, B, K, N, d, ptr(feat), ptr(g.graph_ptr), ptr(minmax), shift, a, b,
+                 ptr(dfeat), stream_ptr())
+        else:
+            dYs = torch.empty(B, K, N, d, dtype=f32, device=dY.device)
+            call("conan_fgw_barycenter_bwd", ptr(T), ptr(_c(dY)), None, None, B, K, N, d, ptr(dYs), stream_ptr())
+            call("conan_fgw_densify_bwd", ptr(feat), ptr(dYs), ptr(g.graph_ptr), ptr(minmax), B * K, N, d, shift, a, b, ptr(dfeat), stream_ptr())
+        return (dfeat,) + (None,) * 8
+
+
+def fgw_densify_barycenter(feat: Tensor, graph: RadiusGraph, batch_size: int, num_conformers: int, max_nodes: int, shift: float,
+                           a: float = 0.1, b: float = 2.0):
+    N, d = int(max_nodes), feat.shape[1]
+    can = lib().conan_fgw_feat_supported(N, d, 0, 1, 0) if feat.is_cuda else 0
+    if can & 1 and (FGW_FUSED_DENSIFY or (FGW_FUSED_BACKWARD and can & 2)):
+        Y, C, T, info, errs, Ys, _ = _DensifyBarycenterFn.apply(feat, graph, int(batch_size), int(num_conformers), N, float(shift), float(a),
+                                                                float(b), dict(PROD_FGW))
+        return Y, C, T, info, errs, Ys
+    Ys, _ = fgw_densify(feat, graph, N, shift, a, b, adjacency=False)
+    Y, C, T, info, errs = fgw_barycenter_batched(Ys.view(batch_size, num_conformers, N, d), None, adjacency=graph)
+    return Y, C, T, info, errs, Ys
+
+
 def fgw_barycenter_batched(Ys: Tensor, Cs: Tensor, ps: Optional[Tensor] = None, p: Optional[Tensor] = None,
                            lambdas: Optional[Tensor] = None, init_C: Optional[Tensor] = None, init_Y: Optional[Tensor] = None,
                            **params):
diff --git a/conan-fgw_amd/schnet.py b/conan-fgw_amd/schnet.py
--- a/conan-fgw_amd/schnet.py
+++ b/conan-fgw_amd/schnet.py
@@ -216,9 +216,7 @@
         if max_nodes is None:
             gp = graph.graph_ptr
             max_nodes = int((gp[1:] - gp[:-1]).max().item())
-        Ys, _ = ops.fgw_densify(node_feature, graph, max_nodes, self.FEATURE_SHIFT, adjacency=False)
-        N, d = max_nodes, node_feature.shape[1]
-        Y, C, T, info, errs = ops.fgw_barycenter_batched(Ys.view(batch_size, K, N, d), None, adjacency=graph)
+        Y, C, T, info, errs, Ys = ops.fgw_densify_barycenter(node_feature, graph, batch_size, K, max_nodes, self.FEATURE_SHIFT)
         self.last_fgw = dict(Y=Y, C=C, T=T, info=info, errs=errs, Ys=Ys)
         return Y, graph
 
diff --git a/include/conan_fgw_hip.h b/include/conan_fgw_hip.h
--- a/include/conan_fgw_hip.h
+++ b/include/conan_fgw_hip.h
@@ -291,6 +291,16 @@
                                     const conan_fgw_params *params , int solver, int symmetric, float *Y, float *C, float *T,
                                     float *T_iter, int *info, float *errs, void *workspace, void *stream);
 
+int conan_fgw_densify_deferred(const float *feat, const int *graph_ptr, int num_graphs, int N, int d, float shift, float a, float b, float *Ys,
+                               float *minmax);
+int conan_fgw_feat_supported(int N, int d, int solver, int symmetric, int loss_fun);
+int conan_fgw_barycenter_prologue_ragged(const float *Ys, const int *graph_ptr, const int *rowptr, const int *col, const int *tgt, const float *ps,
+                                         const float *p, const float *lambdas, const float *init_C, const float *init_Y, int B, int K, int N,
+                                         int d, const conan_fgw_params *params , int solver, int symmetric, float *Y, float *C,
+                                         float *T, float *T_iter, int *info, float *errs, void *workspace, void *stream);
+long long conan_fgw_workspace_order_offset(int B, int K, int N, int d, int ragged, int solver, int symmetric);
+int conan_fgw_set_order_scan(int on);
+
 long long conan_fgw_pair_workspace_bytes(int B, int N, int solver, int symmetric);
 int conan_fgw_pair_fwd(const float *M, const float *C1, const float *C2, const float *p, const float *q, const float *G0, int B, int N,
                        const conan_fgw_params *params , int solver, int symmetric, float *T, float *fgw_dist, int *info,
@@ -319,6 +329,10 @@
 
 int conan_fgw_barycenter_bwd(const float *T, const float *dY, const float *p, const float *lambdas, int B, int K,
                              int N, int d, float *dYs, void *stream);
+
+int conan_fgw_barycenter_bwd_feat(const float *T, const float *dY, const float *p, const float *lambdas, int B, int K, int N, int d,
+                                  const float *feat, const int *graph_ptr, const float *minmax, float shift, float a, float b, float *dfeat,
+                                  void *stream);
 
 long long conan_fgw_barycenter_bwd_full_workspace_bytes(int B, int K, int N, int d);
 int conan_fgw_barycenter_bwd_full(const float *T, const float *Ys, const float *Cs, const float *Y, const float *C, const float *dY,
```

New measurement: 116,700 (median of 6 runs). No clear change (+0.4%).
